# GewelsJI/MVLT

Measured on AMD Instinct MI355X. Metric: image-text pairs/sec/node, PVT-tiny MVLT pre-train step, higher is better.
Workload: dtype bf16

## Files before the change

### mvlt_amd/_lib.py

```python
import ctypes as C
import os

import torch

_HERE = os.path.dirname(os.path.abspath(__file__))
LIB_PATH = os.environ.get("MVLT_HIP_LIB") or os.path.join(_HERE, "libmvlt_hip.so")


class MVLTError(RuntimeError):
    pass


if not os.path.exists(LIB_PATH):
    raise ImportError(f"{LIB_PATH} is missing: build it with `python -m mvlt_amd.build` (hipcc, gfx950). "
                      "mvlt_amd has no CPU or eager fallback.")
lib = C.CDLL(LIB_PATH)

c_int, c_float, c_void_p, c_long = C.c_int, C.c_float, C.c_void_p, C.c_long


class RowMap(C.Structure):
    _fields_ = [(n, c_int) for n in ("mode", "rows_per_batch", "batch_stride", "offset",
                                     "r", "w_in", "tokens_in", "hw_out", "w_out", "c_seg", "h_in")]


class GemmNTArgs(C.Structure):
    _fields_ = [("A", c_void_p), ("B", c_void_p), ("C", c_void_p),
                ("M", c_int), ("N", c_int), ("K", c_int), ("lda", c_int), ("ldb", c_int), ("ldc", c_int),
                ("dtype", c_int), ("out_dtype", c_int),
                ("a_map", RowMap), ("c_map", RowMap),
                ("bias", c_void_p), ("act", c_int), ("H", c_void_p),
                ("row_scale", c_void_p), ("rows_per_scale", c_int), ("R", c_void_p),
                ("col_sum", c_void_p), ("col_sumsq", c_void_p), ("col_copies", c_int), ("split_k", c_int),
                ("post_y", c_void_p), ("post_ld", c_int), ("post_gamma", c_void_p), ("post_beta", c_void_p), ("post_eps", c_float),
                ("post_mean", c_void_p), ("post_rstd", c_void_p), ("r_fp32", c_int)]


class PrepDesc(C.Structure):
    _fields_ = [("src", c_void_p), ("dst", c_void_p), ("kind", c_int), ("R", c_int), ("C", c_int), ("ld_out", c_int),
                ("d0", c_int), ("d1", c_int), ("d2", c_int), ("src_off", c_int), ("ss0", c_int), ("ss1", c_int), ("ss2", c_int),
                ("ds0", c_int), ("ds1", c_int), ("ds2", c_int)]


class GemmTNArgs(C.Structure):
    _fields_ = [("A", c_void_p), ("B", c_void_p), ("C", c_void_p),
                ("M", c_int), ("N1", c_int), ("N2", c_int), ("lda", c_int), ("ldb", c_int), ("ldc", c_int),
                ("dtype", c_int), ("a_map", RowMap), ("b_map", RowMap),
                ("colsum_a", c_void_p), ("splits", c_int), ("colsum_b", c_void_p), ("trans_c", c_int),
                ("c_taps", c_int), ("c_seg", c_int), ("dgrad_wt", c_void_p), ("dgrad_out", c_void_p), ("dgrad_ld", c_int),
                ("partials", c_void_p), ("partials_bytes", c_long), ("defer_fold", c_int), ("c_overwrite", c_int)]


class LayerNormArgs(C.Structure):
    _fields_ = [("x", c_void_p), ("y", c_void_p), ("gamma", c_void_p), ("beta", c_void_p),
                ("mean", c_void_p), ("rstd", c_void_p), ("add", c_void_p), ("add_rows", c_int),
                ("rows", c_int), ("C", c_int), ("ldx", c_int), ("ldy", c_int),
                ("x_map", RowMap), ("y_map", RowMap), ("eps", c_float), ("dtype", c_int), ("y_dtype", c_int),
                ("y2", c_void_p), ("gamma2", c_void_p), ("beta2", c_void_p), ("eps2", c_float), ("mean2", c_void_p), ("rstd2", c_void_p)]


class LayerNormBwdArgs(C.Structure):
    _fields_ = [("dy", c_void_p), ("x", c_void_p), ("dx", c_void_p),
                ("gamma", c_void_p), ("mean", c_void_p), ("rstd", c_void_p),
                ("dgamma", c_void_p), ("dbeta", c_void_p),
                ("rows", c_int), ("C", c_int), ("lddy", c_int), ("ldx", c_int), ("lddx", c_int),
                ("dy_map", RowMap), ("x_map", RowMap), ("dx_map", RowMap),
                ("dx_accumulate", c_int), ("dtype", c_int), ("x_dtype", c_int), ("dx_dtype", c_int),
                ("dx2", c_void_p), ("dx2_scale", c_void_p), ("dx2_rows_per_scale", c_int), ("lddx2", c_int),
                ("dg_copies", c_int), ("dg_copy_stride", c_long)]


class AttnArgs(C.Structure):
    _fields_ = [("Q", c_void_p), ("KV", c_void_p), ("O", c_void_p), ("lse", c_void_p),
                ("B", c_int), ("H", c_int), ("N", c_int), ("M", c_int),
                ("ldq", c_int), ("ldkv", c_int), ("ldo", c_int), ("k_off", c_int), ("v_off", c_int),
                ("scale", c_float), ("dtype", c_int)]


class AttnBwdArgs(C.Structure):
    _fields_ = [("Q", c_void_p), ("KV", c_void_p), ("O", c_void_p), ("dO", c_void_p), ("lse", c_void_p),
                ("dQ", c_void_p), ("dKV", c_void_p),
                ("B", c_int), ("H", c_int), ("N", c_int), ("M", c_int),
                ("ldq", c_int), ("ldkv", c_int), ("ldo", c_int), ("lddkv", c_int),
                ("k_off", c_int), ("v_off", c_int), ("scale", c_float), ("dtype", c_int), ("dkv_dtype", c_int)]


class MlpArgs(C.Structure):
    _fields_ = [("x", c_void_p), ("dy", c_void_p), ("w1", c_void_p), ("wb", c_void_p), ("wc", c_void_p),
                ("b1", c_void_p), ("b2", c_void_p), ("residual", c_void_p), ("row_scale", c_void_p), ("rows_per_scale", c_int),
                ("out", c_void_p), ("h_out", c_void_p), ("dw1", c_void_p), ("db1", c_void_p), ("dw2", c_void_p), ("db2", c_void_p),
                ("M", c_int), ("C", c_int), ("hid", c_int),
                ("ln_x", c_void_p), ("ln_gamma", c_void_p), ("ln_beta", c_void_p), ("ln_eps", c_float),
                ("ln_y", c_void_p), ("ln_mean", c_void_p), ("ln_rstd", c_void_p), ("out_op", c_void_p),
                ("post_gamma", c_void_p), ("post_beta", c_void_p), ("post_eps", c_float),
                ("post_y", c_void_p), ("post_mean", c_void_p), ("post_rstd", c_void_p),
                ("lnb_x", c_void_p), ("lnb_mean", c_void_p), ("lnb_rstd", c_void_p), ("lnb_gamma", c_void_p),
                ("lnb_dx", c_void_p), ("lnb_dx2", c_void_p), ("lnb_dx2_scale", c_void_p), ("lnb_dx2_rows_per_scale", c_int),
                ("lnb_partials", c_void_p), ("partials", c_void_p), ("partials_bytes", c_long), ("defer_fold", c_int)]


STRUCTS = (("mvlt_rowmap", RowMap), ("mvlt_prep_desc", PrepDesc), ("mvlt_gemm_nt_args", GemmNTArgs), ("mvlt_gemm_tn_args", GemmTNArgs),
           ("mvlt_layernorm_args", LayerNormArgs), ("mvlt_layernorm_bwd_args", LayerNormBwdArgs),
           ("mvlt_attn_args", AttnArgs), ("mvlt_attn_bwd_args", AttnBwdArgs), ("mvlt_mlp_args", MlpArgs))

_vp, _i, _l, _f, _u64, _str = c_void_p, c_int, c_long, c_float, C.c_uint64, C.c_char_p
_by_args = lambda cls: (_i, [C.POINTER(cls), _vp])
PROTOTYPES = {
    "mvlt_last_error": (_str, []),
    "mvlt_abi_version": (_i, []),
    "mvlt_last_kernel": (_str, []),
    "mvlt_sizeof": (_i, [_str]),
    "mvlt_gemm_nt": _by_args(GemmNTArgs),
    "mvlt_gemm_tn": _by_args(GemmTNArgs),
    "mvlt_tn_fold_flush": (_i, [_vp, _vp]),
    "mvlt_tn_fold_discard": (_i, [_vp]),
    "mvlt_layernorm_fwd": _by_args(LayerNormArgs),
    "mvlt_layernorm_bwd": _by_args(LayerNormBwdArgs),
    "mvlt_fold_copies": (_i, [_vp, _i, _l, _vp, _i, _i, _vp, _vp]),
    "mvlt_batch_sum": (_i, [_vp, _vp, _i, _i, _i, _l, _i, _i, _vp, _i, _vp]),
    "mvlt_sr_attention_fwd": _by_args(AttnArgs),
    "mvlt_sr_attention_bwd": _by_args(AttnBwdArgs),
    "mvlt_sr_attention_bwd_chunks": (_i, [_i] * 5),
    "mvlt_sr_attention_fwd_streamed": _by_args(AttnArgs),
    "mvlt_sr_attention_bwd_streamed": _by_args(AttnBwdArgs),
    "mvlt_bert_embed_fwd": (_i, [_vp] * 7 + [_f, _vp, _vp, _vp, _i, _i, _i, _f, _i, _vp]),
    "mvlt_bert_embed_bwd": (_i, [_vp] * 7 + [_f] + [_vp] * 7 + [_i, _i, _i, _i, _vp]),
    "mvlt_patchify": (_i, [_vp, _vp, _i, _i, _i, _i, _i, _i, _vp]),
    "mvlt_masked_select": (_i, [_vp, _i, _l, _vp, _vp, _vp]),
    "mvlt_resize_bilinear_tokens": (_i, [_vp, _i, _vp, _i, _i, _i, _i, _i, _i, _i, _vp]),
    "mvlt_resize_bilinear_tokens_multi": (_i, [_vp] * 9 + [_i, _i, _vp]),
    "mvlt_gelu_bwd": (_i, [_vp, _vp, _vp, _l, _i, _vp]),
    "mvlt_loss_compose": (_i, [C.POINTER(c_void_p), C.POINTER(c_float), _vp, _vp, _vp]),
    "mvlt_grid_mask_flags": (_i, [_vp, _i, _i, _i, _i, _i, _u64, _u64, _vp]),
    "mvlt_grid_mask_apply": (_i, [_vp, _vp, _vp, _i, _i, _i, _i, _i, _f, _vp]),
    "mvlt_token_mask": (_i, [_vp, _vp, _vp, _i, _i, _u64, _u64, _i, _vp]),
    "mvlt_keep_mask": (_i, [_vp, _l, _f, _u64, _u64, _vp]),
    "mvlt_droppath_scales": (_i, [_vp, _vp, _i, _i, _u64, _u64, _vp]),
    "mvlt_gather_rows": (_i, [_vp, _vp, _vp, _i, _i, _i, C.POINTER(RowMap), _i, _vp]),
    "mvlt_scatter_rows": (_i, [_vp, _vp, _vp, _i, _i, _i, C.POINTER(RowMap), _i, _i, _vp]),
    "mvlt_cross_entropy_fwd": (_i, [_vp, _vp, _l, _vp, _vp, _vp, _i, _i, _i, _i, _vp]),
    "mvlt_cross_entropy_bwd": (_i, [_vp, _vp, _l, _vp, _vp, _vp, _vp, _i, _i, _i, _i, _i, _i, _vp]),
    "mvlt_smooth_l1_fwd": (_i, [_vp, _vp, _l, _vp, _vp]),
    "mvlt_smooth_l1_bwd": (_i, [_vp, _vp, _l, _vp, _vp, _vp]),
    "mvlt_adamw_step": (_i, [_vp, _vp, _vp, _vp, _vp, _l, _vp, _vp, _vp, _vp]),
    "mvlt_grad_sumsq": (_i, [_vp, _l, _vp, _vp, _i, _vp]),
    "mvlt_clip_coef": (_i, [_vp, _i, _f, _f, _vp, _vp]),
    "mvlt_scale_by_dev": (_i, [_vp, _l, _vp, _vp]),
    "mvlt_cast_bf16": (_i, [_vp, _vp, _l, _vp]),
    "mvlt_row_scale": (_i, [_vp, _vp, _i, _l, _i, _vp, _i, _vp]),
    "mvlt_head_grad_prep": (_i, [_vp, _i, _i, _i, _vp, _vp, _vp, _i, _vp]),
    "mvlt_transpose_cast": (_i, [_vp, _vp, _i, _i, _i, _i, _vp]),
    "mvlt_weight_prep": (_i, [_vp, _vp, _i, _i, _vp, _i, _vp]),
    "mvlt_mlp_fwd": _by_args(MlpArgs),
    "mvlt_mlp_bwd_dx": _by_args(MlpArgs),
    "mvlt_mlp_bwd_dw": _by_args(MlpArgs),
    "mvlt_add_column_sums": (_i, [_vp, _l, _i, _i, _vp, _i, _vp, _vp]),
    "mvlt_col_stats": (_i, [_vp, _i, _l, _i, _vp, _vp, _vp]),
    "mvlt_bn_finalize": (_i, [_vp, _vp, _i, _l, _i, _f, _f, _vp, _vp, _vp, _vp, _vp]),
    "mvlt_bn_norm": (_i, [_vp, _i, _i, _vp, _vp, _vp, _vp, _l, _i, _vp, _i, _i, _vp, _i, _i, _vp]),
    "mvlt_bn_finalize_norm": (_i, [_vp, _i, _vp, _vp, _i, _f, _f, _vp, _vp, _vp, _vp, _vp, _vp, _l, _i, _vp, _i, _i, _vp, _i, _vp]),
    "mvlt_bn_bwd_reduce": (_i, [_vp, _i, _vp, _i, _i, _vp, _vp, _l, _i, _vp, _vp, _i, _vp]),
    "mvlt_bn_bwd_apply": (_i, [_vp, _i, _vp, _i, _i, _vp, _vp, _vp, _vp, _vp, _l, _i, _vp, _i, _vp, _vp, _i, _i, _vp]),
    "mvlt_ew_mul": (_i, [_vp, _i, _vp, _i, _vp, _i, _vp, _i, _i, _l, _i, _i, _vp, _i, _i, _vp]),
    "mvlt_ew_mul3_bwd": (_i, [_vp, _i, _vp, _vp, _vp, _i, _i, _vp, _vp, _vp, _l, _i, _i, _vp]),
    "mvlt_upsample_fwd": (_i, [_vp, _i, _i, _i, _i, _i, _i, _vp, _i, _i, _i, _vp]),
    "mvlt_upsample_bwd": (_i, [_vp, _i, _i, _i, _i, _i, _i, _i, _vp, _i, _i, _i, _i, _vp]),
    "mvlt_upsample_l1_fwd": (_i, [_vp, _i, _i, _i, _i, _i, _i, _vp, _vp, _vp]),
    "mvlt_upsample_l1_bwd": (_i, [_vp, _i, _i, _i, _i, _i, _i, _vp, _vp, _vp, _i, _i, _vp]),
}
EXPORTS = list(PROTOTYPES)
for _name, (_res, _args) in PROTOTYPES.items():
    _fn = getattr(lib, _name)
    _fn.restype, _fn.argtypes = _res, _args

ABI_VERSION = 8
if lib.mvlt_abi_version() != ABI_VERSION:
    raise ImportError(f"ABI mismatch: {LIB_PATH} is version {lib.mvlt_abi_version()}, the binding is version {ABI_VERSION} (stale build? run python -m mvlt_amd.build)")
for _name, _cls in STRUCTS:
    _n = lib.mvlt_sizeof(_name.encode())
    if _n != C.sizeof(_cls):
        raise ImportError(f"ABI mismatch for {_name}: library says {_n} bytes, binding has {C.sizeof(_cls)}")

EXT_PROTOTYPES = {
    "mvlt_ext_version": (_i, []),
    "mvlt_step_gate": (_i, [_vp, _i, _f, _f, _vp, _vp, _vp]),
    "mvlt_adamw_step_gated": (_i, [_vp, _vp, _vp, _vp, _vp, _l, _vp, _vp, _vp, _vp]),
}
for _name, (_res, _args) in EXT_PROTOTYPES.items():
    if not hasattr(lib, _name):
        raise ImportError(f"{LIB_PATH} does not export {_name} (include/mvlt_hip_ext.h): stale build? run python -m mvlt_amd.build")
    _fn = getattr(lib, _name)
    _fn.restype, _fn.argtypes = _res, _args

EXT_VERSION = 1
if lib.mvlt_ext_version() != EXT_VERSION:
    raise ImportError(f"extension mismatch: {LIB_PATH} is version {lib.mvlt_ext_version()}, the binding is version {EXT_VERSION} (stale build? run python -m mvlt_amd.build)")

EMA_PROTOTYPES = {
    "mvlt_ema_version": (_i, []),
    "mvlt_ema_update": (_i, [_vp, _vp, _vp, _l, _f, _f, _vp, _vp]),
    "mvlt_ema_update_buffers": (_i, [_vp, _i, _f, _f, _vp]),
}
for _name, (_res, _args) in EMA_PROTOTYPES.items():
    if not hasattr(lib, _name):
        raise ImportError(f"{LIB_PATH} does not export {_name} (include/mvlt_hip_ema.h): stale build? run python -m mvlt_amd.build")
    _fn = getattr(lib, _name)
    _fn.restype, _fn.argtypes = _res, _args

EMA_VERSION = 1
if lib.mvlt_ema_version() != EMA_VERSION:
    raise ImportError(f"EMA entry points mismatch: {LIB_PATH} is version {lib.mvlt_ema_version()}, the binding is version {EMA_VERSION} (stale build? run python -m mvlt_amd.build)")

class GemmPlan(C.Structure):
    _fields_ = [("family", c_int), ("tp", c_int * 6), ("grid", c_int * 3), ("block", c_int), ("lds", c_int),
                ("ns_flags", c_int), ("nbuf", c_int), ("per_split", c_int), ("t1", c_int), ("t2", c_int), ("splits", c_int),
                ("swap_operands", c_int), ("fold", c_int), ("fold_grid", c_int), ("partials_need", c_long)]


class AttnPlan(C.Structure):
    _fields_ = [("family", c_int), ("tp", c_int * 4), ("grid", c_int), ("block", c_int), ("lds", c_int), ("nq_chunks", c_int), ("q_per_wg", c_int)]


class MlpPlan(C.Structure):
    _fields_ = [("family", c_int), ("tp", c_int * 2), ("grid", c_int), ("block", c_int), ("lds", c_int), ("m_per_split", c_int), ("splits", c_int), ("ny", c_int),
                ("fold", c_int), ("fold_grid", c_int * 2), ("partials_need", c_long)]


PLAN_STRUCTS = (("mvlt_gemm_plan", GemmPlan), ("mvlt_attn_plan", AttnPlan), ("mvlt_mlp_plan", MlpPlan))
PLAN_PROTOTYPES = {
    "mvlt_plan_version": (_i, []),
    "mvlt_gemm_nt_plan": (_i, [C.POINTER(GemmNTArgs), C.POINTER(GemmPlan)]),
    "mvlt_gemm_tn_plan": (_i, [C.POINTER(GemmTNArgs), C.POINTER(GemmPlan)]),
    "mvlt_gemm_plan_name": (_i, [C.POINTER(GemmPlan), _str, C.c_size_t]),
    "mvlt_gemm_plan_sizeof": (_i, []),
    "mvlt_sr_attention_fwd_plan": (_i, [C.POINTER(AttnArgs), _i, C.POINTER(AttnPlan)]),
    "mvlt_sr_attention_bwd_plan": (_i, [C.POINTER(AttnBwdArgs), _i, C.POINTER(AttnPlan)]),
    "mvlt_attn_plan_name": (_i, [C.POINTER(AttnPlan), _str, C.c_size_t]),
    "mvlt_attn_plan_sizeof": (_i, []),
    "mvlt_mlp_fwd_plan": (_i, [C.POINTER(MlpArgs), C.POINTER(MlpPlan)]),
    "mvlt_mlp_bwd_dx_plan": (_i, [C.POINTER(MlpArgs), C.POINTER(MlpPlan)]),
    "mvlt_mlp_bwd_dw_plan": (_i, [C.POINTER(MlpArgs), C.POINTER(MlpPlan)]),
    "mvlt_mlp_plan_name": (_i, [C.POINTER(MlpPlan), _str, C.c_size_t]),
    "mvlt_mlp_plan_sizeof": (_i, []),
}
for _name, (_res, _args) in PLAN_PROTOTYPES.items():
    if not hasattr(lib, _name):
        raise ImportError(f"{LIB_PATH} does not export {_name} (include/mvlt_hip_plan.h): stale build? run python -m mvlt_amd.build")
    _fn = getattr(lib, _name)
    _fn.restype, _fn.argtypes = _res, _args

PLAN_VERSION = 3
_plan_sizes = [(n, getattr(lib, n + "_sizeof")(), C.sizeof(c)) for n, c in PLAN_STRUCTS]
if lib.mvlt_plan_version() != PLAN_VERSION or any(have != want for _, have, want in _plan_sizes):
    raise ImportError(f"plan entry points mismatch: {LIB_PATH} is version {lib.mvlt_plan_version()}, the binding is version {PLAN_VERSION}; (struct, bytes in the library, "
                      f"bytes in the binding): {_plan_sizes} (stale build? run python -m mvlt_amd.build)")

OPT_PROTOTYPES = {
    "mvlt_opt_version": (_i, []),
    "mvlt_adamw_step_groups": (_i, [_vp, _vp, _vp, _vp, _vp, _l, _vp, _vp, _vp, _i, _vp, _vp, _vp]),
}
for _name, (_res, _args) in OPT_PROTOTYPES.items():
    if not hasattr(lib, _name):
        raise ImportError(f"{LIB_PATH} does not export {_name} (include/mvlt_hip_opt.h): stale build? run python -m mvlt_amd.build")
    _fn = getattr(lib, _name)
    _fn.restype, _fn.argtypes = _res, _args

OPT_VERSION = 1
if lib.mvlt_opt_version() != OPT_VERSION:
    raise ImportError(f"optimizer entry points mismatch: {LIB_PATH} is version {lib.mvlt_opt_version()}, the binding is version {OPT_VERSION} (stale build? run python -m mvlt_amd.build)")

LAMB_PROTOTYPES = {
    "mvlt_lamb_version": (_i, []),
    "mvlt_lamb_check_tables": (_i, [_vp, _i, _vp, _i, _l, _i]),
    "mvlt_lamb_moments": (_i, [_vp, _vp, _vp, _vp, _l, _vp, _vp, _i, _vp, _i, _vp, _i, _vp, _vp, _vp, _vp]),
    "mvlt_lamb_fold": (_i, [_vp, _i, _vp, _i, _vp, _i, _i, _vp, _vp, _vp]),
    "mvlt_lamb_apply": (_i, [_vp, _vp, _vp, _vp, _l, _vp, _vp, _i, _vp, _i, _vp, _i, _vp, _vp, _vp]),
}
for _name, (_res, _args) in LAMB_PROTOTYPES.items():
    if not hasattr(lib, _name):
        raise ImportError(f"{LIB_PATH} does not export {_name} (include/mvlt_hip_lamb.h): stale build? run python -m mvlt_amd.build")
    _fn = getattr(lib, _name)
    _fn.restype, _fn.argtypes = _res, _args

LAMB_VERSION = 1
if lib.mvlt_lamb_version() != LAMB_VERSION:
    raise ImportError(f"LAMB entry points mismatch: {LIB_PATH} is version {lib.mvlt_lamb_version()}, the binding is version {LAMB_VERSION} (stale build? run python -m mvlt_amd.build)")

LOSS_PROTOTYPES = {
    "mvlt_loss_version": (_i, []),
    "mvlt_ce_smooth_fwd": (_i, [_vp, _vp, _l, _f, _vp, _vp, _vp, _vp, _i, _i, _i, _i, _vp]),
    "mvlt_ce_smooth_bwd": (_i, [_vp, _vp, _l, _f, _vp, _vp, _vp, _vp, _vp, _i, _i, _i, _i, _i, _i, _vp]),
}
for _name, (_res, _args) in LOSS_PROTOTYPES.items():
    if not hasattr(lib, _name):
        raise ImportError(f"{LIB_PATH} does not export {_name} (include/mvlt_hip_loss.h): stale build? run python -m mvlt_amd.build")
    _fn = getattr(lib, _name)
    _fn.restype, _fn.argtypes = _res, _args

LOSS_VERSION = 1
if lib.mvlt_loss_version() != LOSS_VERSION:
    raise ImportError(f"loss entry points mismatch: {LIB_PATH} is version {lib.mvlt_loss_version()}, the binding is version {LOSS_VERSION} (stale build? run python -m mvlt_amd.build)")

INGEST_PROTOTYPES = {
    "mvlt_ingest_version": (_i, []),
    "mvlt_image_ingest": (_i, [_vp, _i, _vp, _vp, _vp, _vp, _i, _i, _i, _i, _f, _vp]),
    "mvlt_image_ingest_resize": (_i, [_vp, _i, _i, _vp, _vp, _vp, _vp, _vp, _vp, _vp, _i, _i, _i, _i, _f, _vp]),
    "mvlt_flip_flags": (_i, [_vp, _i, _f, _u64, _u64, _vp]),
}
for _name, (_res, _args) in INGEST_PROTOTYPES.items():
    if not hasattr(lib, _name):
        raise ImportError(f"{LIB_PATH} does not export {_name} (include/mvlt_hip_ingest.h): stale build? run python -m mvlt_amd.build")
    _fn = getattr(lib, _name)
    _fn.restype, _fn.argtypes = _res, _args

INGEST_VERSION = 1
if lib.mvlt_ingest_version() != INGEST_VERSION:
    raise ImportError(f"ingest entry points mismatch: {LIB_PATH} is version {lib.mvlt_ingest_version()}, the binding is version {INGEST_VERSION} (stale build? run python -m mvlt_amd.build)")

DT = {torch.bfloat16: 0, torch.float32: 1}


def last_kernel():
    s = lib.mvlt_last_kernel().decode()
    s = s.replace("(anonymous namespace)::", "")
    if s.startswith("void "):
        s = s[5:]
    depth = 0
    for i, ch in enumerate(s):
        depth += ch == "<"
        depth -= ch == ">"
        if ch == "(" and depth == 0:
            return s[:i]
    return s


def check(rc, what):
    if rc != 0:
        raise MVLTError(f"{what} failed ({rc}): {lib.mvlt_last_error().decode()}")


_raw_stream, _cur_device = torch._C._cuda_getCurrentRawStream, torch._C._cuda_getDevice


def stream_ptr():
    return _raw_stream(_cur_device())


def ptr(t):
    if t is None:
        return None
    if not t.is_cuda:
        raise MVLTError("mvlt_amd ops need CUDA/HIP tensors (no CPU fallback)")
    return t.data_ptr()


def rowmap(rows_per_batch=0, batch_stride=0, offset=0):
    return RowMap(0, rows_per_batch, batch_stride, offset, 0, 0, 0, 0, 0, 0, 0)


def patchmap(r, w_in, tokens_in, hw_out, w_out, c_seg):
    return RowMap(1, 0, 0, 0, r, w_in, tokens_in, hw_out, w_out, c_seg, 0)


def conv3map(h, w, tokens_in, c_seg):
    return RowMap(2, 0, 0, 0, 3, w, tokens_in, h * w, w, c_seg, h)
```

### mvlt_amd/build.py

```python
import concurrent.futures
import os
import subprocess
import sys

HERE = os.path.dirname(os.path.abspath(__file__))
CSRC = os.path.join(HERE, "csrc")
OBJ = os.path.join(HERE, "csrc", "_obj")
LIB = os.path.join(HERE, "libmvlt_hip.so")
ARCH = "gfx950"
FLAGS = ["--offload-arch=" + ARCH, "-O3", "-std=c++17", "-fPIC", "-ffp-contract=fast", "-Wno-unused-result"]
EXTRA = {f: ["-fno-slp-vectorize"] for f in ("mlp_fused.hip", "mlp_pipe.hip", "mlp_wgrad.hip")}


def _sources():
    return sorted(f for f in os.listdir(CSRC) if f.endswith(".hip"))


def source_hash():
    import hashlib
    h = hashlib.sha256()
    files = sorted(os.path.join(CSRC, f) for f in os.listdir(CSRC) if f.endswith((".hip", ".h", ".inc")))
    files += [os.path.join(HERE, "..", "include", h) for h in ("mvlt_hip.h", "mvlt_hip_ext.h", "mvlt_hip_ema.h", "mvlt_hip_plan.h", "mvlt_hip_opt.h", "mvlt_hip_lamb.h", "mvlt_hip_loss.h", "mvlt_hip_ingest.h")]
    for f in files:
        h.update(os.path.basename(f).encode())
        h.update(open(f, "rb").read())
    return h.hexdigest()[:16]


def _deps_mtime():
    hdrs = [os.path.join(CSRC, f) for f in os.listdir(CSRC) if f.endswith((".h", ".inc"))]
    hdrs += [os.path.join(HERE, "..", "include", h) for h in ("mvlt_hip.h", "mvlt_hip_ext.h", "mvlt_hip_ema.h", "mvlt_hip_plan.h", "mvlt_hip_opt.h", "mvlt_hip_lamb.h", "mvlt_hip_loss.h", "mvlt_hip_ingest.h")]
    return max(os.path.getmtime(h) for h in hdrs)


def _compile(src, force, verbose):
    s = os.path.join(CSRC, src)
    o = os.path.join(OBJ, src[:-4] + ".o")
    if not force and os.path.exists(o) and os.path.getmtime(o) >= max(os.path.getmtime(s), _deps_mtime()):
        return o
    cmd = ["hipcc", *FLAGS, *EXTRA.get(src, []), "-c", s, "-o", o]
    if verbose:
        print(" ".join(cmd), flush=True)
    r = subprocess.run(cmd, capture_output=True, text=True)
    if r.returncode != 0:
        raise RuntimeError(f"hipcc failed for {src}:\n{r.stdout}\n{r.stderr}")
    return o


def build(force=False, verbose=False):
    os.makedirs(OBJ, exist_ok=True)
    srcs = _sources()
    with concurrent.futures.ThreadPoolExecutor(max_workers=min(8, len(srcs))) as ex:
        objs = list(ex.map(lambda s: _compile(s, force, verbose), srcs))
    if force or not os.path.exists(LIB) or any(os.path.getmtime(o) > os.path.getmtime(LIB) for o in objs):
        cmd = ["hipcc", "--offload-arch=" + ARCH, "-shared", "-fPIC", *objs, "-o", LIB]
        if verbose:
            print(" ".join(cmd), flush=True)
        r = subprocess.run(cmd, capture_output=True, text=True)
        if r.returncode != 0:
            raise RuntimeError(f"link failed:\n{r.stdout}\n{r.stderr}")
    return LIB


if __name__ == "__main__":
    print(build(force="--force" in sys.argv, verbose="--verbose" in sys.argv or True))
```

### mvlt_amd/csrc/gemm.hip

```cpp
#include "gemm_common.h"
#include <map>
#include <mutex>

namespace {

constexpr int FOLD_MAX = 32;
struct FoldDesc { const bf16* part; float* C; int splits, N1, N2, ldc, wg0; };
struct FoldBatch { FoldDesc d[FOLD_MAX]; int n, total_wgs; };

__device__ __forceinline__ void tn_fold_body(const bf16* __restrict__ part, int splits, int N1, int N2, float* __restrict__ C, int ldc, int blk) {
  __shared__ float red[8][32][9];
  const int eg = threadIdx.x & 31, sk = threadIdx.x >> 5;
  const long g = (long)blk * 32 + eg;
  const long per = (long)N1 * N2;
  const bool ok = g * 8 < per;
  float s[8] = {0.f, 0.f, 0.f, 0.f, 0.f, 0.f, 0.f, 0.f};
  if (ok) {
    for (int z = sk; z < splits; z += 8) {
      const bf16x8 v = __builtin_bit_cast(bf16x8, ld_g<MVLT_NT_LD>((const u32x4*)(part + (size_t)z * per + g * 8)));
#pragma unroll
      for (int e = 0; e < 8; ++e) s[e] += (float)v[e];
    }
  }
#pragma unroll
  for (int e = 0; e < 8; ++e) red[sk][eg][e] = s[e];
  __syncthreads();
  if (sk == 0 && ok) {
#pragma unroll
    for (int k = 1; k < 8; ++k)
#pragma unroll
      for (int e = 0; e < 8; ++e) s[e] += red[k][eg][e];
    const int n1 = (int)((g * 8) / N2), n2 = (int)((g * 8) - (long)n1 * N2);
    float* dst = C + (long)n1 * ldc + n2;
    const f32x4 a = *(const f32x4*)dst, b = *(const f32x4*)(dst + 4);
    *(f32x4*)dst = f32x4{a[0] + s[0], a[1] + s[1], a[2] + s[2], a[3] + s[3]};
    *(f32x4*)(dst + 4) = f32x4{b[0] + s[4], b[1] + s[5], b[2] + s[6], b[3] + s[7]};
  }
}

__global__ __launch_bounds__(256) void tn_fold_kernel(const bf16* __restrict__ part, int splits, int N1, int N2, float* __restrict__ C, int ldc) {
  tn_fold_body(part, splits, N1, N2, C, ldc, blockIdx.x);
}
__global__ __launch_bounds__(256) void tn_fold_multi_kernel(FoldBatch b) {
  int i = 0;
#pragma unroll 1
  for (int k = 1; k < b.n; ++k) if ((int)blockIdx.x >= b.d[k].wg0) i = k;
  const FoldDesc& d = b.d[i];
  tn_fold_body(d.part, d.splits, d.N1, d.N2, d.C, d.ldc, (int)blockIdx.x - d.wg0);
}

struct FoldPending {
  FoldBatch b = {};
  long used = 0;
  hipStream_t stream = nullptr;
  hipEvent_t ev = nullptr;
};
std::mutex g_fold_mu;
std::map<const void*, FoldPending> g_fold;
int fold_wgs(const FoldDesc& d) { return (int)(((long)d.N1 * d.N2 / 8 + 31) / 32); }
void fold_flush_locked(FoldPending& f, hipStream_t reader, bool order_reader) {
  if (f.b.n > 0) {
    f.b.total_wgs = f.b.d[f.b.n - 1].wg0 + fold_wgs(f.b.d[f.b.n - 1]);
    MVLT_LAUNCH(tn_fold_multi_kernel, dim3((unsigned)f.b.total_wgs), dim3(256), 0, f.stream, f.b);
    if (order_reader && reader != f.stream) {
      if (!f.ev) (void)hipEventCreateWithFlags(&f.ev, hipEventDisableTiming);
      if (f.ev && hipEventRecord(f.ev, f.stream) == hipSuccess) (void)hipStreamWaitEvent(reader, f.ev, 0);
    }
  }
  f.b.n = 0;
  f.used = 0;
}
bf16* fold_acquire(const mvlt_gemm_tn_args& a, long need, hipStream_t s, int room = 1) {
  if (!a.partials || ((uintptr_t)a.partials & 15) || need > a.partials_bytes) return nullptr;
  std::lock_guard<std::mutex> lk(g_fold_mu);
  FoldPending& f = g_fold[a.partials];
  bool flush = f.b.n > 0 && (!a.defer_fold || f.stream != s || f.b.n + room > FOLD_MAX || f.used + need > a.partials_bytes);
  const float* c_lo = a.C;
  const float* c_hi = a.C + (size_t)(a.N1 - 1) * a.ldc + a.N2;
  for (int i = 0; i < f.b.n && !flush; ++i) {
    const FoldDesc& d = f.b.d[i];
    const float* d_lo = d.C;
    const float* d_hi = d.C + (size_t)(d.N1 - 1) * d.ldc + d.N2;
    if (c_lo < d_hi && d_lo < c_hi) flush = true;
  }
  if (flush) fold_flush_locked(f, s, true);
  f.stream = s;
  if (!a.defer_fold) return (bf16*)a.partials;
  return (bf16*)((char*)a.partials + f.used);
}
void fold_launch(const mvlt_gemm_tn_args& a, const bf16* part, int splits, hipStream_t s) {
  const long groups = (long)a.N1 * a.N2 / 8;
  if (!a.defer_fold) {
    MVLT_LAUNCH(tn_fold_kernel, dim3((unsigned)((groups + 31) / 32)), dim3(256), 0, s, part, splits, a.N1, a.N2, a.C, a.ldc);
    return;
  }
  std::lock_guard<std::mutex> lk(g_fold_mu);
  FoldPending& f = g_fold[a.partials];
  FoldDesc& d = f.b.d[f.b.n];
  d.part = part; d.C = a.C; d.splits = splits; d.N1 = a.N1; d.N2 = a.N2; d.ldc = a.ldc;
  d.wg0 = f.b.n == 0 ? 0 : f.b.d[f.b.n - 1].wg0 + fold_wgs(f.b.d[f.b.n - 1]);
  ++f.b.n;
  f.used += ((long)splits * a.N1 * a.N2 * 2 + 255) & ~255L;
}

int launch_nt(const mvlt_gemm_plan& p, const mvlt_gemm_nt_args& a, hipStream_t s) {
  switch (p.family) {
    case MVLT_GEMM_NT_F32:
    case MVLT_GEMM_NT_DMA: return mvlt_launch_nt_dma(p, a, s);
    case MVLT_GEMM_NT_P8: return mvlt_launch_nt_p8(p, a, s);
    case MVLT_GEMM_NT_CONV3: return mvlt_launch_nt_conv3(p, a, s);
  }
  return no_instantiation("mvlt_gemm_nt", p);
}

int launch_tn(const mvlt_gemm_plan& p, const mvlt_gemm_tn_args& a, hipStream_t s) {
  const char* const who = "mvlt_gemm_tn";
  mvlt_gemm_tn_args k = a;
  if (p.swap_operands) {
    k.A = a.B; k.B = a.A; k.lda = a.ldb; k.ldb = a.lda; k.N1 = a.N2; k.N2 = a.N1;
    k.colsum_a = a.colsum_b; k.colsum_b = a.colsum_a;
  }
  bf16* const part = p.fold ? fold_acquire(a, p.partials_need, s) : nullptr;
  if (p.fold && !part) { mvlt_set_error("%s: the planned %ld bytes of partial tiles do not fit the scratch", who, p.partials_need); return MVLT_ERR_ARG; }
  auto launch = [&]() -> int {
    switch (p.family) {
      case MVLT_GEMM_TN_PLAIN:
      case MVLT_GEMM_TN_DMA: return mvlt_launch_tn_dma(p, k, part, s);
      case MVLT_GEMM_TN_P8: return mvlt_launch_tn_p8(p, k, part, s);
      case MVLT_GEMM_TN_CONV3: return mvlt_launch_tn_conv3(p, k, part, s);
    }
    return no_instantiation(who, p);
  };
  const int e = launch();
  if (e != MVLT_OK || !p.fold) return e;
  fold_launch(a, part, p.splits, s);
  return mvlt_check_launch(who);
}
}

extern "C" int mvlt_gemm_nt(const mvlt_gemm_nt_args* a, void* stream) {
  mvlt_gemm_plan p;
  MVLT_REQUIRE(a, "mvlt_gemm_nt: null operand");
  if (int e = plan_gemm_nt(*a, p)) return e;
  return p.family == MVLT_GEMM_NONE ? MVLT_OK : launch_nt(p, *a, (hipStream_t)stream);
}

extern "C" int mvlt_gemm_tn(const mvlt_gemm_tn_args* a, void* stream) {
  mvlt_gemm_plan p;
  MVLT_REQUIRE(a, "mvlt_gemm_tn: null operand");
  if (int e = plan_gemm_tn(*a, p)) return e;
  return p.family == MVLT_GEMM_NONE ? MVLT_OK : launch_tn(p, *a, (hipStream_t)stream);
}

extern "C" int mvlt_plan_version(void) { return MVLT_PLAN_VERSION; }
extern "C" int mvlt_gemm_plan_sizeof(void) { return (int)sizeof(mvlt_gemm_plan); }
extern "C" int mvlt_gemm_nt_plan(const mvlt_gemm_nt_args* a, mvlt_gemm_plan* plan) {
  MVLT_REQUIRE(a && plan, "mvlt_gemm_nt_plan: null argument");
  return plan_gemm_nt(*a, *plan);
}
extern "C" int mvlt_gemm_tn_plan(const mvlt_gemm_tn_args* a, mvlt_gemm_plan* plan) {
  MVLT_REQUIRE(a && plan, "mvlt_gemm_tn_plan: null argument");
  return plan_gemm_tn(*a, *plan);
}
extern "C" int mvlt_gemm_plan_name(const mvlt_gemm_plan* plan, char* buf, size_t n) {
  MVLT_REQUIRE(plan && buf && n > 0, "mvlt_gemm_plan_name: null argument");
  return plan_kernel_name(*plan, buf, n);
}

bf16* mvlt_fold_acquire_ext(const mvlt_gemm_tn_args& a, long need, hipStream_t s, int descriptors) { return fold_acquire(a, need, s, descriptors); }
void mvlt_fold_launch_ext(const mvlt_gemm_tn_args& a, const bf16* part, int splits, hipStream_t s) { fold_launch(a, part, splits, s); }

extern "C" int mvlt_tn_fold_discard(const void* partials) {
  std::lock_guard<std::mutex> lk(g_fold_mu);
  for (auto& kv : g_fold)
    if (!partials || kv.first == partials) { kv.second.b.n = 0; kv.second.used = 0; }
  return MVLT_OK;
}

extern "C" int mvlt_tn_fold_flush(const void* partials, void* stream) {
  std::lock_guard<std::mutex> lk(g_fold_mu);
  for (auto& kv : g_fold)
    if (!partials || kv.first == partials) fold_flush_locked(kv.second, (hipStream_t)stream, true);
  return mvlt_check_launch("mvlt_tn_fold_flush");
}
```

### mvlt_amd/csrc/gemm_common.h

```cpp
#pragma once
#include "common.h"
#include "gemm_plan.h"
#include <type_traits>
#include "../../include/mvlt_hip.h"

int mvlt_launch_nt_dma(const mvlt_gemm_plan& p, const mvlt_gemm_nt_args& a, hipStream_t s);
int mvlt_launch_nt_p8(const mvlt_gemm_plan& p, const mvlt_gemm_nt_args& a, hipStream_t s);
int mvlt_launch_nt_conv3(const mvlt_gemm_plan& p, const mvlt_gemm_nt_args& a, hipStream_t s);
int mvlt_launch_tn_dma(const mvlt_gemm_plan& p, const mvlt_gemm_tn_args& k, bf16* part, hipStream_t s);
int mvlt_launch_tn_p8(const mvlt_gemm_plan& p, const mvlt_gemm_tn_args& k, bf16* part, hipStream_t s);
int mvlt_launch_tn_conv3(const mvlt_gemm_plan& p, const mvlt_gemm_tn_args& k, bf16* part, hipStream_t s);

namespace {

constexpr int BM = 128;
constexpr int NTHREADS = 256;
constexpr int ROW_BYTES = 128;
constexpr int CHUNKS = 8;

template <typename T> struct Elem;
template <> struct Elem<bf16> { static constexpr int BK = 64; static constexpr int PER_CHUNK = 8; };
template <> struct Elem<float> { static constexpr int BK = 32; static constexpr int PER_CHUNK = 4; };

__device__ __forceinline__ int swz(int row, int chunk) { return chunk ^ ((row >> 1) & 7); }

__device__ __forceinline__ RowMap to_rowmap(const mvlt_rowmap& m) {
  RowMap r;
  r.mode = m.mode; r.rows_per_batch = m.rows_per_batch; r.batch_stride = m.batch_stride; r.offset = m.offset;
  r.r = m.r; r.w_in = m.w_in; r.tokens_in = m.tokens_in; r.hw_out = m.hw_out; r.w_out = m.w_out; r.c_seg = m.c_seg;
  r.h_in = m.h_in;
  return r;
}

__device__ __forceinline__ void mma16(f32x4& acc, const u32x4& a0, const u32x4& a1, const u32x4& b0, const u32x4& b1, bf16*) {
  acc = __builtin_amdgcn_mfma_f32_16x16x32_bf16(__builtin_bit_cast(bf16x8, a0), __builtin_bit_cast(bf16x8, b0), acc, 0, 0, 0);
  (void)a1; (void)b1;
}
__device__ __forceinline__ void mma16(f32x4& acc, const u32x4& a0, const u32x4& a1, const u32x4& b0, const u32x4& b1, float*) {
  f32x4 fa0 = __builtin_bit_cast(f32x4, a0), fa1 = __builtin_bit_cast(f32x4, a1);
  f32x4 fb0 = __builtin_bit_cast(f32x4, b0), fb1 = __builtin_bit_cast(f32x4, b1);
#pragma unroll
  for (int j = 0; j < 4; ++j) acc = __builtin_amdgcn_mfma_f32_16x16x4f32(fa0[j], fb0[j], acc, 0, 0, 0);
#pragma unroll
  for (int j = 0; j < 4; ++j) acc = __builtin_amdgcn_mfma_f32_16x16x4f32(fa1[j], fb1[j], acc, 0, 0, 0);
}

typedef _Float16 f16x8 __attribute__((ext_vector_type(8)));
__device__ __forceinline__ void round_f16_8(float (&v)[8]) {
#pragma unroll
  for (int e = 0; e < 8; ++e) v[e] = (float)(_Float16)__builtin_amdgcn_fmed3f(v[e], -65504.f, 65504.f);
}
template <bool NTF> __device__ __forceinline__ void store_f16_8(void* base, long ix, const float (&v)[8]) {
  f16x8 o;
#pragma unroll
  for (int e = 0; e < 8; ++e) o[e] = (_Float16)v[e];
  st_g<NTF>((f16x8*)((_Float16*)base + ix), o);
}
template <typename T> __device__ __forceinline__ void store_out(void* base, long idx, float v, int out_fp32) {
  if (out_fp32) ((float*)base)[idx] = v; else ((bf16*)base)[idx] = (bf16)v;
}
__device__ __forceinline__ float load_out(const void* base, long idx, int out_fp32) {
  return out_fp32 ? ((const float*)base)[idx] : (float)((const bf16*)base)[idx];
}

template <typename T, int BN>
__device__ __forceinline__ void nt_epilogue(const mvlt_gemm_nt_args& p, f32x4 (&acc)[4][BN / 32], char* smem, int m0, int n0,
                                            int wave, int lane) {
  constexpr int WN = BN / 2;
  constexpr int TN_ = WN / 16;
  const int wm = wave >> 1, wn = wave & 1;
  const int fr = lane & 15, fg = lane >> 4;
  const RowMap cmap = to_rowmap(p.c_map);
  const int ofp32 = p.out_dtype;
  constexpr int LDW = WN + 4;
  constexpr int CPR = WN / 8;
  constexpr int RPI = 64 / CPR;
  float* stage = (float*)smem + wave * 32 * LDW;
  const bool vec_ok = (p.ldc % 8 == 0) && (((uintptr_t)p.C & 15) == 0) && (!p.R || ((uintptr_t)p.R & 15) == 0) &&
                      (!p.H || ((uintptr_t)p.H & 15) == 0);
  const int nc_lane = n0 + wn * WN + (lane % CPR) * 8;
  float bias8[8];
#pragma unroll
  for (int e = 0; e < 8; ++e) bias8[e] = 0.f;
  if (p.bias && p.split_k <= 1) {
    if (nc_lane + 8 <= p.N && (((uintptr_t)p.bias & 15) == 0)) {
      f32x4 b0 = *(const f32x4*)(p.bias + nc_lane), b1 = *(const f32x4*)(p.bias + nc_lane + 4);
#pragma unroll
      for (int e = 0; e < 4; ++e) { bias8[e] = b0[e]; bias8[4 + e] = b1[e]; }
    } else {
#pragma unroll
      for (int e = 0; e < 8; ++e) if (nc_lane + e < p.N) bias8[e] = p.bias[nc_lane + e];
    }
  }
  float cs8[8], cq8[8];
#pragma unroll
  for (int e = 0; e < 8; ++e) { cs8[e] = 0.f; cq8[e] = 0.f; }
#pragma unroll
  for (int half = 0; half < 2; ++half) {
    __builtin_amdgcn_wave_barrier();
#pragma unroll
    for (int ii = 0; ii < 2; ++ii)
#pragma unroll
      for (int j = 0; j < TN_; ++j)
#pragma unroll
        for (int r = 0; r < 4; ++r) stage[(ii * 16 + 4 * fg + r) * LDW + j * 16 + fr] = acc[half * 2 + ii][j][r];
    __builtin_amdgcn_fence(__ATOMIC_RELEASE, "wavefront");
    __builtin_amdgcn_wave_barrier();
    __builtin_amdgcn_fence(__ATOMIC_ACQUIRE, "wavefront");
    if (p.split_k > 1) {
      const int col = n0 + wn * WN + lane;
      if (lane < WN && col < p.N) {
        const float bv = (p.bias && blockIdx.y == 0) ? p.bias[col] : 0.f;
        for (int r = 0; r < 32; ++r) {
          const int m = m0 + wm * 64 + half * 32 + r;
          if (m < p.M) atomicAdd((float*)p.C + (long)m * p.ldc + col, stage[r * LDW + lane] + bv);
        }
      }
      continue;
    }
#pragma unroll
    for (int it = 0; it < 32 / RPI; ++it) {
      const int rl = it * RPI + lane / CPR;
      const int ch = lane % CPR;
      const int m = m0 + wm * 64 + half * 32 + rl;
      const int nc = n0 + wn * WN + ch * 8;
      if (m >= p.M || nc >= p.N) continue;
      f32x4 v0 = *(const f32x4*)(stage + rl * LDW + ch * 8), v1 = *(const f32x4*)(stage + rl * LDW + ch * 8 + 4);
      float v[8] = {v0[0], v0[1], v0[2], v0[3], v1[0], v1[1], v1[2], v1[3]};
      int seg_rows = 0, ncol = nc;
      if (cmap.mode == 1) {
        int seg = nc / cmap.c_seg;
        ncol = nc - seg * cmap.c_seg;
        seg_rows = rowmap_seg(cmap, seg);
      }
      const long idx = (rowmap_base(cmap, m) + seg_rows) * p.ldc + ncol;
      const bool full = vec_ok && (nc + 8 <= p.N);
      const float rs = p.row_scale ? p.row_scale[m / p.rows_per_scale] : 1.0f;
#pragma unroll
      for (int e = 0; e < 8; ++e) v[e] += bias8[e];
      if (full) {
        auto load8 = [&](const void* base, float* o) {
          if (ofp32) {
            f32x4 a = *(const f32x4*)((const float*)base + idx), b = *(const f32x4*)((const float*)base + idx + 4);
#pragma unroll
            for (int e = 0; e < 4; ++e) { o[e] = a[e]; o[4 + e] = b[e]; }
          } else {
            bf16x8 a = *(const bf16x8*)((const bf16*)base + idx);
#pragma unroll
            for (int e = 0; e < 8; ++e) o[e] = (float)a[e];
          }
        };
        auto store8 = [&](void* base, const float* o) {
          if (ofp32) {
            st_g<MVLT_NT_GEMM>((f32x4*)((float*)base + idx), f32x4{o[0], o[1], o[2], o[3]});
            st_g<MVLT_NT_GEMM>((f32x4*)((float*)base + idx + 4), f32x4{o[4], o[5], o[6], o[7]});
          } else {
            bf16x8 a;
#pragma unroll
            for (int e = 0; e < 8; ++e) a[e] = (bf16)o[e];
            st_g<MVLT_NT_GEMM>((bf16x8*)((bf16*)base + idx), a);
          }
        };
        if (p.act == 1) {
          if (p.H) store8(p.H, v);
#pragma unroll
          for (int e = 0; e < 8; e += 2) {
            const f32x2 gv = gelu_erf2(f32x2{v[e], v[e + 1]});
            v[e] = gv[0]; v[e + 1] = gv[1];
          }
        } else if (p.act == 2) {
          float h8[8];
          load8(p.H, h8);
#pragma unroll
          for (int e = 0; e < 8; e += 2) {
            const f32x2 dv = gelu_erf_grad2(f32x2{h8[e], h8[e + 1]});
            v[e] *= dv[0]; v[e + 1] *= dv[1];
          }
        }
        if (p.row_scale) {
#pragma unroll
          for (int e = 0; e < 8; ++e) v[e] *= rs;
        }
        if (p.R) {
          float r8[8];
          load8(p.R, r8);
#pragma unroll
          for (int e = 0; e < 8; ++e) v[e] += r8[e];
        }
        if (p.col_sum) {
#pragma unroll
          for (int e = 0; e < 8; ++e) { cs8[e] += v[e]; cq8[e] += v[e] * v[e]; }
        }
        store8(p.C, v);
      } else {
        for (int e = 0; e < 8; ++e) {
          if (nc + e >= p.N) break;
          float x = v[e];
          if (p.act == 1) {
            if (p.H) store_out<T>(p.H, idx + e, x, ofp32);
            x = gelu_erf(x);
          } else if (p.act == 2) {
            x *= gelu_erf_grad(load_out(p.H, idx + e, ofp32));
          }
          x *= rs;
          if (p.R) x += load_out(p.R, idx + e, ofp32);
          if (p.col_sum) { cs8[e] += x; cq8[e] += x * x; }
          store_out<T>(p.C, idx + e, x, ofp32);
        }
      }
    }
  }
  if (p.col_sum) {
#pragma unroll
    for (int off = CPR; off < 64; off <<= 1)
#pragma unroll
      for (int e = 0; e < 8; ++e) { cs8[e] += __shfl_xor(cs8[e], off); cq8[e] += __shfl_xor(cq8[e], off); }
    __builtin_amdgcn_fence(__ATOMIC_RELEASE, "wavefront");
    __builtin_amdgcn_wave_barrier();
    if (lane < CPR) {
#pragma unroll
      for (int e = 0; e < 8; ++e) { stage[lane * 8 + e] = cs8[e]; stage[WN + lane * 8 + e] = cq8[e]; }
    }
    __builtin_amdgcn_fence(__ATOMIC_RELEASE, "wavefront");
    __builtin_amdgcn_wave_barrier();
    __builtin_amdgcn_fence(__ATOMIC_ACQUIRE, "wavefront");
    const int col = n0 + wn * WN + lane;
    const long cpy = p.col_copies > 1 ? (long)((m0 / BM) % p.col_copies) * p.N : 0;
    if (lane < WN && col < p.N) {
      atomicAdd(&p.col_sum[cpy + col], stage[lane]);
      atomicAdd(&p.col_sumsq[cpy + col], stage[WN + lane]);
    }
  }
}

__device__ __forceinline__ int fdiv24(int m, int d, float inv) {
  int q = (int)((float)m * inv);
  int r = m - q * d;
  return q + (r >= d) - (r < 0);
}
template <int BN, int EPIX, int TM = 4, int NWN = 2, bool FULL = false>
__device__ __forceinline__ void nt_epilogue_lean(const mvlt_gemm_nt_args& p, f32x4 (&acc)[TM][BN / 32], char* smem, int m0, int n0,
                                                 int wave, int lane) {
  static_assert(NWN == 2 || EPIX != 8, "the LayerNorm epilogue pairs the two waves of a row: 2 x 2 wave grids only");
  constexpr bool SCAT = (EPIX == 6 || EPIX == 7);
  constexpr bool POST = EPIX == 8;
  constexpr int EPI = EPIX == 6 ? 1 : (EPIX == 7 || EPIX == 8) ? 2 : EPIX;
  constexpr int WN = BN / 2;
  constexpr int TN_ = WN / 16;
  constexpr int LDW = WN + 4;
  constexpr int CPR = WN / 8;
  constexpr int RPI = 64 / CPR;
  constexpr int NIT = 32 / RPI;
  const int wm = wave / NWN, wn = wave % NWN;
  const int fr = lane & 15, fg = lane >> 4;
  const int ofp32 = (EPI == 3 || EPI == 4) ? 0 : p.out_dtype;
  const int rfp32 = (EPI == 2 && !POST) ? (ofp32 | p.r_fp32) : ofp32;
  float* stage = (float*)smem + wave * 32 * LDW;
  const int ch = lane % CPR;
  const int nc = n0 + wn * WN + ch * 8;
  const bool col_ok = FULL || nc < p.N;
  float bias8[8];
#pragma unroll
  for (int e = 0; e < 8; ++e) bias8[e] = 0.f;
  if (p.bias && col_ok) {
    if (!FULL && nc + 8 > p.N) {
#pragma unroll
      for (int e = 0; e < 8; ++e) if (nc + e < p.N) bias8[e] = p.bias[nc + e];
    } else if (((uintptr_t)p.bias & 15) == 0) {
      f32x4 b0 = *(const f32x4*)(p.bias + nc), b1 = *(const f32x4*)(p.bias + nc + 4);
#pragma unroll
      for (int e = 0; e < 4; ++e) { bias8[e] = b0[e]; bias8[4 + e] = b1[e]; }
    } else {
#pragma unroll
      for (int e = 0; e < 8; ++e) bias8[e] = p.bias[nc + e];
    }
  }
  constexpr int NH = TM / 2;
  const int m_first = m0 + wm * (TM * 16) + lane / CPR;
  const int rpb = p.c_map.rows_per_batch;
  const float inv_rpb = rpb > 0 ? 1.0f / (float)rpb : 0.f;
  int seg_rows = 0, ncol = nc;
  float inv_hw = 0.f, inv_w = 0.f;
  if constexpr (SCAT) {
    const int seg = nc / p.c_map.c_seg;
    ncol = nc - seg * p.c_map.c_seg;
    const int di = seg / p.c_map.r;
    seg_rows = di * p.c_map.w_in + (seg - di * p.c_map.r);
    inv_hw = 1.0f / (float)p.c_map.hw_out;
    inv_w = 1.0f / (float)p.c_map.w_out;
  }
  const float inv_rps = (EPI == 2 && p.rows_per_scale > 0) ? 1.0f / (float)p.rows_per_scale : 0.f;
  float cs8[8], cq8[8];
  if (EPI == 5) {
#pragma unroll
    for (int e = 0; e < 8; ++e) { cs8[e] = 0.f; cq8[e] = 0.f; }
  }
  long idx[2][NIT];
  bool ok[2][NIT];
  float rs[2][NIT];
  u32x4 raw[2][NIT][2];
  auto request = [&](int half) {
    const int sl = half & 1;
#pragma unroll
    for (int it = 0; it < NIT; ++it) {
      const int m = m_first + half * 32 + it * RPI;
      ok[sl][it] = FULL || (m < p.M && col_ok);
      const int mm = (FULL || ok[sl][it]) ? m : 0;
      long phys = mm;
      if constexpr (SCAT) {
// ... 500 lines not shown
```

### mvlt_amd/csrc/gemm_nt_dma.hip

```cpp
#include "gemm_common.h"

namespace {

template <typename T, int BN>
__global__ __launch_bounds__(NTHREADS) void gemm_nt_kernel(mvlt_gemm_nt_args p, int nbuf) {
  constexpr int BK = Elem<T>::BK;
  constexpr int PC = Elem<T>::PER_CHUNK;
  constexpr int WN = BN / 2;
  constexpr int TN_ = WN / 16;
  constexpr int A_ITERS = BM * CHUNKS / NTHREADS;
  constexpr int B_ITERS = BN * CHUNKS / NTHREADS;
  extern __shared__ __attribute__((aligned(16))) char smem[];
  char* sA = smem;
  char* sB = smem + nbuf * BM * ROW_BYTES;

  const int tid = threadIdx.x, lane = tid & 63, wave = tid >> 6;
  const int wm = wave >> 1, wn = wave & 1;
  const int tiles_m = (p.M + BM - 1) / BM;
  const int tiles_n = (p.N + BN - 1) / BN;
  const int bid = blockIdx.x;
  const int xcd = bid & 7, slot = bid >> 3;
  const int tile_m = (slot / tiles_n) * 8 + xcd, tile_n = slot % tiles_n;
  if (tile_m >= tiles_m) return;
  const int m0 = tile_m * BM, n0 = tile_n * BN;
  const RowMap amap = to_rowmap(p.a_map);

  const int chunk = tid & 7;
  const int row_in = tid >> 3;
  const T* Ag = (const T*)p.A;
  const T* Bg = (const T*)p.B;

  long a_base[A_ITERS];
  bool a_ok[A_ITERS];
  int a_y[A_ITERS], a_x[A_ITERS];
#pragma unroll
  for (int i = 0; i < A_ITERS; ++i) {
    int m = m0 + row_in + 32 * i;
    a_ok[i] = m < p.M;
    a_base[i] = a_ok[i] ? rowmap_base(amap, m) : 0;
    a_y[i] = 0; a_x[i] = 0;
    if (amap.mode == 2 && a_ok[i]) rowmap_yx(amap, m, a_y[i], a_x[i]);
  }
  long b_base[B_ITERS];
  bool b_ok[B_ITERS];
#pragma unroll
  for (int i = 0; i < B_ITERS; ++i) {
    int n = n0 + row_in + 32 * i;
    b_ok[i] = n < p.N;
    b_base[i] = b_ok[i] ? (long)n * p.ldb : 0;
  }

  u32x4 ra[A_ITERS], rb[B_ITERS];
  auto gload = [&](int kt) {
    const int k = kt * BK + chunk * PC;
    const bool k_ok = k < p.K;
    int seg_rows = 0, kk = k, seg = 0;
    if (amap.mode != 0) {
      seg = k / amap.c_seg;
      kk = k - seg * amap.c_seg;
      if (amap.mode == 1) seg_rows = rowmap_seg(amap, seg);
    }
#pragma unroll
    for (int i = 0; i < A_ITERS; ++i) {
      u32x4 v = {0u, 0u, 0u, 0u};
      bool ok = a_ok[i] && k_ok;
      int off = seg_rows;
      if (amap.mode == 2) ok = ok && rowmap_nb(amap, seg, a_y[i], a_x[i], off);
      if (ok) v = *(const u32x4*)(Ag + (a_base[i] + off) * p.lda + kk);
      ra[i] = v;
    }
#pragma unroll
    for (int i = 0; i < B_ITERS; ++i) {
      u32x4 v = {0u, 0u, 0u, 0u};
      if (b_ok[i] && k_ok) v = *(const u32x4*)(Bg + b_base[i] + k);
      rb[i] = v;
    }
  };
  auto lstore = [&](int buf) {
#pragma unroll
    for (int i = 0; i < A_ITERS; ++i) {
      int r = row_in + 32 * i;
      *(u32x4*)(sA + buf * BM * ROW_BYTES + r * ROW_BYTES + swz(r, chunk) * 16) = ra[i];
    }
#pragma unroll
    for (int i = 0; i < B_ITERS; ++i) {
      int r = row_in + 32 * i;
      *(u32x4*)(sB + buf * BN * ROW_BYTES + r * ROW_BYTES + swz(r, chunk) * 16) = rb[i];
    }
  };

  f32x4 acc[4][TN_];
#pragma unroll
  for (int i = 0; i < 4; ++i)
#pragma unroll
    for (int j = 0; j < TN_; ++j) acc[i][j] = f32x4{0.f, 0.f, 0.f, 0.f};

  const int nk = (p.K + BK - 1) / BK;
  gload(0);
  lstore(0);
  __syncthreads();
  const int fr = lane & 15, fg = lane >> 4;
  for (int kt = 0; kt < nk; ++kt) {
    const int buf = kt & 1;
    if (kt + 1 < nk) gload(kt + 1);
    const char* a_s = sA + buf * BM * ROW_BYTES + (wm * 64) * ROW_BYTES;
    const char* b_s = sB + buf * BN * ROW_BYTES + (wn * WN) * ROW_BYTES;
    constexpr int KSTEPS = (sizeof(T) == 2) ? 2 : 1;
    constexpr int CPS = (sizeof(T) == 2) ? 1 : 2;
#pragma unroll
    for (int ks = 0; ks < KSTEPS; ++ks) {
      u32x4 fa[4][2], fb[TN_][2];
#pragma unroll
      for (int i = 0; i < 4; ++i) {
        int r = i * 16 + fr;
        int rr = wm * 64 + r;
#pragma unroll
        for (int c = 0; c < CPS; ++c) {
          int ch = (sizeof(T) == 2) ? (ks * 4 + fg) : (fg * 2 + c);
          fa[i][c] = *(const u32x4*)(a_s + r * ROW_BYTES + swz(rr, ch) * 16);
        }
        if (CPS == 1) fa[i][1] = fa[i][0];
      }
#pragma unroll
      for (int j = 0; j < TN_; ++j) {
        int r = j * 16 + fr;
        int rr = wn * WN + r;
#pragma unroll
        for (int c = 0; c < CPS; ++c) {
          int ch = (sizeof(T) == 2) ? (ks * 4 + fg) : (fg * 2 + c);
          fb[j][c] = *(const u32x4*)(b_s + r * ROW_BYTES + swz(rr, ch) * 16);
        }
        if (CPS == 1) fb[j][1] = fb[j][0];
      }
#pragma unroll
      for (int i = 0; i < 4; ++i)
#pragma unroll
        for (int j = 0; j < TN_; ++j) mma16(acc[i][j], fa[i][0], fa[i][1], fb[j][0], fb[j][1], (T*)nullptr);
    }
    if (kt + 1 < nk) lstore(buf ^ 1);
    __syncthreads();
  }

  nt_epilogue<T, BN>(p, acc, smem, m0, n0, wave, lane);
}

template <int BN, int AMODE, int EPI, int BK, int BMT = BM>
__global__ __launch_bounds__(NTHREADS, BMT == 256 ? 2 : 1) void gemm_nt_dma_kernel(mvlt_gemm_nt_args p, int ns_flags) {
  const int ns = ns_flags & 0xff;
  const bool early = (ns_flags & 0x100) != 0;
  constexpr int ROWB = BK * 2;
  constexpr int CH = BK / 8;
  constexpr int RPL = NTHREADS / CH;
  constexpr int WN = BN / 2, TN_ = WN / 16;
  constexpr int WM = BMT / 2, TM_ = WM / 16;
  constexpr int A_ITERS = BMT * CH / NTHREADS;
  constexpr int B_ITERS = BN * CH / NTHREADS;
  constexpr int LPT = A_ITERS + B_ITERS;
  constexpr int STAGE = (BMT + BN) * ROWB;
  auto swzk = [](int row, int chunk) { return CH == 8 ? (chunk ^ ((row >> 1) & 7)) : (chunk ^ ((0 - (row >> 2)) & 3)); };
  extern __shared__ __attribute__((aligned(16))) char smem[];

  const int tid = threadIdx.x, lane = tid & 63, wave = __builtin_amdgcn_readfirstlane(tid >> 6);
  const int wm = wave >> 1, wn = wave & 1;
  const int tiles_m = (p.M + BMT - 1) / BMT;
  const int tiles_n = (p.N + BN - 1) / BN;
  const int bid = blockIdx.x;
  const int xcd = bid & 7, bslot = bid >> 3;
  const int tile_m = (bslot / tiles_n) * 8 + xcd, tile_n = bslot % tiles_n;
  if (tile_m >= tiles_m) return;
  const int m0 = tile_m * BMT, n0 = tile_n * BN;
  const RowMap amap = to_rowmap(p.a_map);
  const unsigned smem_lds = (unsigned)(uintptr_t)smem;

  const int row_in = tid / CH;
  const int chunk = swzk(row_in, tid % CH);
  const char* zsrc = (const char*)g_zero_page + ((tid * 16 + (bid & 15) * 4096) & 65535);

  const char* a_ptr[A_ITERS];
  bool a_ok[A_ITERS];
  int a_y[A_ITERS], a_x[A_ITERS];
#pragma unroll
  for (int i = 0; i < A_ITERS; ++i) {
    int m = m0 + row_in + RPL * i;
    a_ok[i] = m < p.M;
    RowIt it = row_init(amap, a_ok[i] ? m : 0);
    int phys;
    if constexpr (AMODE == 0) phys = it.b * amap.batch_stride + amap.offset + it.x;
    else if constexpr (AMODE == 1) phys = it.b * amap.tokens_in + (it.y * amap.r) * amap.w_in + it.x * amap.r;
    else phys = it.b * amap.tokens_in + it.y * amap.w_in + it.x;
    a_y[i] = it.y; a_x[i] = it.x;
    a_ptr[i] = (const char*)p.A + (unsigned long long)(unsigned)phys * (2u * (unsigned)p.lda);
  }
  const char* b_ptr[B_ITERS];
  bool b_ok[B_ITERS];
#pragma unroll
  for (int i = 0; i < B_ITERS; ++i) {
    int n = n0 + row_in + RPL * i;
    b_ok[i] = n < p.N;
    b_ptr[i] = (const char*)p.B + (unsigned long long)(unsigned)(b_ok[i] ? n : 0) * (2u * (unsigned)p.ldb);
  }

  const int nk_all = (p.K + BK - 1) / BK;
  const int nsplit = p.split_k > 1 ? p.split_k : 1;
  const int kt_per = (nk_all + nsplit - 1) / nsplit;
  const int kt0 = blockIdx.y * kt_per;
  int kpos = kt0 * BK + chunk * 8, seg = 0, kk = kpos;
  if constexpr (AMODE != 0) { seg = kk / amap.c_seg; kk -= seg * amap.c_seg; }
  auto issue = [&](int slot) {
    const bool k_ok = kpos < p.K;
    int off_bytes = (AMODE == 0 ? kpos : kk) * 2, tdy = 0, tdx = 0;
    if constexpr (AMODE == 1) off_bytes += rowmap_seg(amap, seg) * (2 * p.lda);
    if constexpr (AMODE == 2) {
      const int dy = seg / 3;
      tdy = dy - 1; tdx = seg - dy * 3 - 1;
      off_bytes += (tdy * amap.w_in + tdx) * (2 * p.lda);
    }
#pragma unroll
    for (int i = 0; i < A_ITERS; ++i) {
      bool ok = a_ok[i] && k_ok;
      if constexpr (AMODE == 2) ok = ok && (unsigned)(a_y[i] + tdy) < (unsigned)amap.h_in && (unsigned)(a_x[i] + tdx) < (unsigned)amap.w_in;
      glds16(ok ? a_ptr[i] + off_bytes : zsrc, __builtin_amdgcn_readfirstlane(smem_lds + slot * STAGE + (i * NTHREADS + wave * 64) * 16));
    }
#pragma unroll
    for (int i = 0; i < B_ITERS; ++i)
      glds16((b_ok[i] && k_ok) ? b_ptr[i] + kpos * 2 : zsrc,
             __builtin_amdgcn_readfirstlane(smem_lds + slot * STAGE + BMT * ROWB + (i * NTHREADS + wave * 64) * 16));
    kpos += BK;
    if constexpr (AMODE != 0) {
      kk += BK;
      while (kk >= amap.c_seg) { kk -= amap.c_seg; ++seg; }
    }
  };

  f32x4 acc[TM_][TN_];
#pragma unroll
  for (int i = 0; i < TM_; ++i)
#pragma unroll
    for (int j = 0; j < TN_; ++j) acc[i][j] = f32x4{0.f, 0.f, 0.f, 0.f};

  const int nk = min(kt_per, nk_all - kt0);
  if (nk <= 0) return;
  const int fr = lane & 15, fg = lane >> 4;
  for (int st = 0; st < (early ? ns : ns - 1) && st < nk; ++st) issue(st);
  if (ns == 1 && !early) issue(0);
  int slot = 0, islot = early ? 0 : ns - 1;
  for (int kt = 0; kt < nk; ++kt) {
    const int ahead = min(nk - 1 - kt, early ? ns - 1 : ns - 2);
    if (ahead >= 4) asm volatile("s_waitcnt vmcnt(%0) lgkmcnt(0)" ::"n"(4 * LPT) : "memory");
    else if (ahead == 3) asm volatile("s_waitcnt vmcnt(%0) lgkmcnt(0)" ::"n"(3 * LPT) : "memory");
    else if (ahead == 2) asm volatile("s_waitcnt vmcnt(%0) lgkmcnt(0)" ::"n"(2 * LPT) : "memory");
    else if (ahead == 1) asm volatile("s_waitcnt vmcnt(%0) lgkmcnt(0)" ::"n"(LPT) : "memory");
    else asm volatile("s_waitcnt vmcnt(0) lgkmcnt(0)" ::: "memory");
    __builtin_amdgcn_s_barrier();
    asm volatile("" ::: "memory");
    if (!early) {
      if (ns > 1 && kt + ns - 1 < nk) issue(islot);
      islot = islot + 1 >= ns ? 0 : islot + 1;
    }
    const char* a_s = smem + slot * STAGE + (wm * WM) * ROWB;
    const char* b_s = smem + slot * STAGE + BMT * ROWB + (wn * WN) * ROWB;
    slot = slot + 1 >= ns ? 0 : slot + 1;
    constexpr int KS = BK / 32;
    u32x4 fa[KS][TM_], fb[KS][TN_];
#pragma unroll
    for (int ks = 0; ks < KS; ++ks) {
#pragma unroll
      for (int i = 0; i < TM_; ++i) {
        int r = i * 16 + fr;
        fa[ks][i] = *(const u32x4*)(a_s + r * ROWB + swzk(wm * WM + r, ks * 4 + fg) * 16);
      }
#pragma unroll
      for (int j = 0; j < TN_; ++j) {
        int r = j * 16 + fr;
        fb[ks][j] = *(const u32x4*)(b_s + r * ROWB + swzk(wn * WN + r, ks * 4 + fg) * 16);
      }
    }
    if (early) {
      asm volatile("s_waitcnt lgkmcnt(0)" ::: "memory");
      __builtin_amdgcn_s_barrier();
      asm volatile("" ::: "memory");
      if (kt + ns < nk) issue(islot);
      islot = islot + 1 >= ns ? 0 : islot + 1;
    }
#pragma unroll
    for (int ks = 0; ks < KS; ++ks) {
      __builtin_amdgcn_sched_barrier(0);
#pragma unroll
      for (int i = 0; i < TM_; ++i)
#pragma unroll
        for (int j = 0; j < TN_; ++j) mma16(acc[i][j], fa[ks][i], fa[ks][i], fb[ks][j], fb[ks][j], (bf16*)nullptr);
    }
  }
  __syncthreads();
  static_assert(BMT == BM || (BN != 192 && EPI != 0), "the 256-row tile carries the lean epilogues only");
  if constexpr (BN == 192) nt_epilogue_192<EPI>(p, acc, smem, m0, n0, wave, lane);
  else if constexpr (EPI == 0) nt_epilogue<bf16, BN>(p, acc, smem, m0, n0, wave, lane);
  else nt_epilogue_lean<BN, EPI, TM_>(p, acc, smem, m0, n0, wave, lane);
}

}

int mvlt_launch_nt_dma(const mvlt_gemm_plan& p, const mvlt_gemm_nt_args& a, hipStream_t s) {
  const char* const who = "mvlt_gemm_nt";
  MVLT_PLAN_LAUNCH_HEAD;
#define NT_F32(BN_) MVLT_CASE(false, (gemm_nt_kernel<float, BN_>), (MVLT_GEMM_NT_F32, BN_), a, p.nbuf)
#define NT_DMA(BN_, AM_, EPI_, BK_) MVLT_CASE(false, (gemm_nt_dma_kernel<BN_, AM_, EPI_, BK_>), (MVLT_GEMM_NT_DMA, BN_, AM_, EPI_, BK_), a, p.ns_flags)
#define NT_DMA_EPIS(BN_, AM_) NT_DMA(BN_, AM_, 1, 64) NT_DMA(BN_, AM_, 2, 64) NT_DMA(BN_, AM_, 3, 64) NT_DMA(BN_, AM_, 4, 64) \
                              NT_DMA(BN_, AM_, 5, 64) NT_DMA(BN_, AM_, 6, 64) NT_DMA(BN_, AM_, 7, 64) NT_DMA(BN_, AM_, 0, 64)
  switch (key) {
    NT_DMA(64, 0, 8, 64) NT_DMA(128, 0, 8, 64)
    NT_DMA(192, 0, 1, 64) NT_DMA(192, 0, 5, 64) NT_DMA(192, 2, 1, 64) NT_DMA(192, 2, 5, 64)
    NT_DMA_EPIS(64, 0) NT_DMA_EPIS(64, 1) NT_DMA_EPIS(64, 2)
    NT_DMA(128, 0, 3, 32) NT_DMA(128, 0, 4, 32)
    NT_DMA_EPIS(128, 0) NT_DMA_EPIS(128, 1) NT_DMA_EPIS(128, 2)
    NT_F32(64) NT_F32(128)
  }
  return no_instantiation(who, p);
}
```

### mvlt_amd/csrc/gemm_plan.h

```cpp
#pragma once
#include <stdint.h>
#include <stdio.h>
#include "../../include/mvlt_hip_plan.h"
#include "plan_common.h"
#ifndef MVLT_NT_EARLY_DEFAULT
#define MVLT_NT_EARLY_DEFAULT 0x100
#endif

namespace mvlt_plan {

constexpr int BM = 128;
constexpr int NTHREADS = 256;
constexpr int ROW_BYTES = 128;
constexpr int TBK = 64;
constexpr int TN_ROWB_BF16 = (TBK + 8) * 2, TN_ROWB_F32 = (TBK + 4) * 4;
constexpr int TN_TILE64_BYTES = TBK * 64 * 2;

inline bool al16(const void* p) { return ((uintptr_t)p & 15) == 0; }
inline int cdiv(int a, int b) { return (a + b - 1) / b; }
inline int xcd_grid(int n) { return n >= 8 ? 8 * cdiv(n, 8) : n; }
inline int xcd_round(int splits) { return splits >= 8 ? (splits + 4) / 8 * 8 : splits; }

struct Split { int splits, per; };
inline Split split_even(int splits, int ktiles) {
  if (splits > ktiles) splits = ktiles;
  if (splits < 1) splits = 1;
  const int per = cdiv(ktiles, splits);
  return {cdiv(ktiles, per), per};
}
inline Split split_choose(int want, int ktiles, int min_tiles, bool round_first) {
  if (round_first) { want = xcd_round(want); if (want > 4096) want = 4096; }
  if (want > ktiles / min_tiles) want = ktiles / min_tiles;
  if (!round_first) want = xcd_round(want);
  return split_even(want, ktiles);
}
inline int fold_workgroups(int N1, int N2) { return (int)(((long)N1 * N2 / 8 + 31) / 32); }
inline bool scratch_fits(const mvlt_gemm_tn_args& a, long need) { return a.partials && al16(a.partials) && need <= a.partials_bytes; }
inline void plan_fold(const mvlt_gemm_tn_args& a, mvlt_gemm_plan& p) {
  p.fold = 1;
  p.partials_need = (long)p.splits * a.N1 * a.N2 * 2;
  p.fold_grid = fold_workgroups(a.N1, a.N2);
}

inline int check_rowmap(const mvlt_rowmap& m, const char* who) {
  if (m.mode == 0) {
    MVLT_REQUIRE(m.rows_per_batch >= 0, "%s: rows_per_batch < 0", who);
  } else if (m.mode == 1) {
    MVLT_REQUIRE(m.r > 0 && m.w_in > 0 && m.tokens_in > 0 && m.hw_out > 0 && m.w_out > 0 && m.c_seg > 0 && m.c_seg % 16 == 0,
                 "%s: bad patch map (c_seg must be a positive multiple of 16)", who);
  } else if (m.mode == 2) {
    MVLT_REQUIRE(m.r == 3 && m.w_in > 0 && m.h_in > 0 && m.tokens_in >= m.h_in * m.w_in && m.hw_out == m.h_in * m.w_in &&
                 m.w_out == m.w_in && m.c_seg > 0 && m.c_seg % 8 == 0, "%s: bad 3x3 neighbourhood map", who);
  } else {
    MVLT_REQUIRE(false, "%s: unknown rowmap mode %d", who, m.mode);
  }
  return MVLT_OK;
}

inline void set_tp(mvlt_gemm_plan& p, int family, int t0, int t1 = 0, int t2 = 0, int t3 = 0, int t4 = 0, int t5 = 0) {
  p.family = family;
  p.tp[0] = t0; p.tp[1] = t1; p.tp[2] = t2; p.tp[3] = t3; p.tp[4] = t4; p.tp[5] = t5;
}
inline void set_launch(mvlt_gemm_plan& p, int gx, int gy, int gz, int block, long lds) {
  p.grid[0] = gx; p.grid[1] = gy; p.grid[2] = gz; p.block = block; p.lds = (int)lds;
}
inline void plan_nt_p8(const mvlt_gemm_nt_args& a, mvlt_gemm_plan& p, int epi, int hm, int hn0, int hn1, int rag) {
  const int bmt = 64 * hm, bnt = 64 * (hn0 + hn1);
  const int lds_loop = 2 * (2 * (2 * hm * 16) + 64 * (hn0 + hn1)) * 128, lds_epi = 8 * 32 * (16 * (hn0 + hn1) + 4) * 4;
  set_tp(p, MVLT_GEMM_NT_P8, epi, hm, hn0, hn1, rag);
  set_launch(p, 8 * cdiv(cdiv(a.M, bmt), 8) * cdiv(a.N, bnt), 1, 1, 512, lds_loop > lds_epi ? lds_loop : lds_epi);
}

}

inline int plan_gemm_nt(const mvlt_gemm_nt_args& a, mvlt_gemm_plan& p) {
  using namespace mvlt_plan;
  p = mvlt_gemm_plan{};
  MVLT_REQUIRE(a.A && a.B && a.C, "mvlt_gemm_nt: null operand");
  MVLT_REQUIRE(a.M >= 0 && a.N > 0 && a.K > 0, "mvlt_gemm_nt: bad shape M=%d N=%d K=%d", a.M, a.N, a.K);
  MVLT_REQUIRE(a.dtype == 0 || a.dtype == 1, "mvlt_gemm_nt: dtype must be 0 (bf16) or 1 (fp32)");
  const int pc = a.dtype == 0 ? 8 : 4;
  MVLT_REQUIRE(a.K % pc == 0 && a.lda % pc == 0 && a.ldb % pc == 0, "mvlt_gemm_nt: K/lda/ldb must be multiples of %d elements (16 B)", pc);
  MVLT_REQUIRE(al16(a.A) && al16(a.B), "mvlt_gemm_nt: A/B must be 16-byte aligned");
  MVLT_REQUIRE(a.act >= 0 && a.act <= 2, "mvlt_gemm_nt: bad act");
  MVLT_REQUIRE(a.act != 2 || a.H, "mvlt_gemm_nt: act=2 (gelu') needs H");
  MVLT_REQUIRE(!a.row_scale || a.rows_per_scale > 0, "mvlt_gemm_nt: row_scale needs rows_per_scale");
  MVLT_REQUIRE((a.col_sum == nullptr) == (a.col_sumsq == nullptr), "mvlt_gemm_nt: col_sum and col_sumsq come together");
  MVLT_REQUIRE(a.split_k <= 1 || (a.dtype == 0 && a.out_dtype == 1 && a.act == 0 && !a.H && !a.R && !a.row_scale && !a.col_sum &&
                                  a.c_map.mode == 0 && a.split_k <= 64),
               "mvlt_gemm_nt: split_k needs bf16 operands, fp32 C (zeroed by the caller) and a plain epilogue (A may be gathered)");
  MVLT_REQUIRE(a.col_copies >= 0, "mvlt_gemm_nt: col_copies < 0");
  MVLT_REQUIRE(!a.r_fp32 || (a.R && a.R != a.C && a.dtype == 0 && a.out_dtype == 0 && a.act == 0 && !a.col_sum && !a.post_y && a.split_k <= 1 && a.c_map.mode == 0 &&
                             a.N % 8 == 0 && a.ldc % 8 == 0 && (((uintptr_t)a.C | (uintptr_t)a.R) & 15) == 0 && a.M < (1 << 24)),
               "mvlt_gemm_nt: r_fp32 (fp32 residual beside a bf16 C) exists in the residual epilogue of the bf16 LDS-DMA kernels only (plain c_map, N % 8 == 0, 16-byte aligned C / R)");
  MVLT_REQUIRE(a.out_dtype >= 0 && a.out_dtype <= 2, "mvlt_gemm_nt: out_dtype is 0 (bf16), 1 (fp32) or 2 (fp16, with col_sum only)");
  MVLT_REQUIRE(a.out_dtype != 2 || (a.dtype == 0 && a.col_sum && a.act == 0 && !a.R && !a.row_scale && a.split_k <= 1 && a.c_map.mode == 0 && a.N % 8 == 0 &&
                                    a.ldc % 8 == 0 && al16(a.C) && a.M < (1 << 24)),
               "mvlt_gemm_nt: fp16 output exists in the column-statistics epilogue of the bf16 LDS-DMA kernels only (plain c_map, N % 8 == 0, 16-byte aligned C)");
  if (int e = check_rowmap(a.a_map, "mvlt_gemm_nt a_map")) return e;
  if (int e = check_rowmap(a.c_map, "mvlt_gemm_nt c_map")) return e;
  MVLT_REQUIRE(a.a_map.mode == 0 || a.K == a.a_map.r * a.a_map.r * a.a_map.c_seg, "mvlt_gemm_nt: gather K != r*r*c_seg");
  MVLT_REQUIRE(a.c_map.mode == 0 || a.N == a.c_map.r * a.c_map.r * a.c_map.c_seg, "mvlt_gemm_nt: scatter N != r*r*c_seg");
  MVLT_REQUIRE(a.c_map.mode != 2, "mvlt_gemm_nt: the 3x3 map is a gather only (its dgrad is a gather with flipped taps)");
  MVLT_REQUIRE(!a.post_y || (a.dtype == 0 && a.split_k <= 1),
               "mvlt_gemm_nt: post_y needs the bf16 LDS-DMA path (no fp32 operands, no split_k)");
  if (a.M == 0) return MVLT_OK;
  const int tiles_m = cdiv(a.M, BM);
  const bool narrow = a.N <= 64;
  const int bn = narrow ? 64 : 128;
  const int tiles_n = cdiv(a.N, bn);
  const int ksplit = a.split_k > 1 ? a.split_k : 1;
  const long stage = (long)4 * 32 * (bn / 2 + 4) * sizeof(float);
  const int gx = 8 * cdiv(tiles_m, 8) * tiles_n;
  if (a.dtype != 0) {
    p.nbuf = a.K <= 32 ? 1 : 2;
    const long lds = (long)p.nbuf * (BM + bn) * ROW_BYTES;
    set_tp(p, MVLT_GEMM_NT_F32, bn);
    set_launch(p, gx, ksplit, 1, NTHREADS, lds < stage ? stage : lds);
    return MVLT_OK;
  }
  int epi = 0;
  const bool plain_epi = a.act == 0 && !a.R && !a.row_scale && !a.col_sum && !a.H && a.c_map.mode == 0;
  const bool lean_ok = (a.c_map.mode == 0 || (a.c_map.mode == 1 && a.c_map.c_seg % 8 == 0)) && a.split_k <= 1 && (a.N % 8 == 0 || plain_epi) && a.ldc % 8 == 0 && al16(a.C) &&
                       (!a.R || al16(a.R)) && (!a.H || al16(a.H)) && a.M < (1 << 24);
  if (lean_ok && a.c_map.mode == 1) {
    if (a.act == 0 && !a.col_sum && !a.R && !a.row_scale) epi = 6;
    else if (a.act == 0 && !a.col_sum && a.R) epi = 7;
  } else if (lean_ok) {
    if (a.act == 1 && !a.R && !a.row_scale && !a.col_sum && a.out_dtype == 0) epi = 3;
    else if (a.act == 2 && !a.R && !a.row_scale && !a.col_sum && a.out_dtype == 0) epi = 4;
    else if (a.act == 0 && a.R && !a.col_sum) epi = 2;
    else if (a.act == 0 && !a.R && !a.row_scale && a.col_sum) epi = 5;
    else if (a.act == 0 && !a.R && !a.row_scale && !a.col_sum) epi = 1;
  }
  const int bk = (!narrow && a.a_map.mode == 0 && (epi == 3 || epi == 4) && a.K <= 512) ? 32 : 64;
  const int nk = bk == 32 ? cdiv(a.K, 32) : cdiv(cdiv(a.K, 64), ksplit);
  const int ns = nk < 2 ? nk : 2;
  p.ns_flags = nk >= 2 ? ns | MVLT_NT_EARLY_DEFAULT : ns;
  long lds = (long)ns * (BM + bn) * (bk * 2);
  if (lds < stage) lds = stage;
  if (a.post_y) {
    MVLT_REQUIRE(epi == 2 && a.N == bn && a.a_map.mode == 0 && a.c_map.mode == 0 && a.c_map.rows_per_batch == 0 && a.post_gamma && a.post_beta &&
                 a.post_mean && a.post_rstd && a.post_ld % 8 == 0 && al16(a.post_y) && al16(a.post_gamma),
                 "mvlt_gemm_nt: post_y needs bf16 operands, a residual (R), N == 64 or 128, identity row maps, 16-byte aligned outputs");
    set_tp(p, MVLT_GEMM_NT_DMA, bn, 0, 8, 64);
    set_launch(p, gx, ksplit, 1, NTHREADS, lds < stage + 2048 ? stage + 2048 : lds);
    return MVLT_OK;
  }
  if (a.a_map.mode == 2 && (epi == 1 || epi == 2 || epi == 5) && a.split_k <= 1 && a.a_map.c_seg % 64 == 0 && a.c_map.mode == 0 &&
      (a.a_map.w_in == 16 || a.a_map.w_in == 32 || a.a_map.w_in == 64) && (a.a_map.h_in * a.a_map.w_in) % BM == 0 && a.M % BM == 0 &&
      a.M % (a.a_map.h_in * a.a_map.w_in) == 0 && a.a_map.hw_out == a.a_map.h_in * a.a_map.w_in && a.a_map.w_out == a.a_map.w_in &&
      a.K == 9 * a.a_map.c_seg && a.lda >= a.a_map.c_seg && a.ldb >= a.K) {
    const int w = a.a_map.w_in;
    const int cbn = (a.N % 192 == 0 && a.N % 128 != 0 && epi != 2) ? 192 : a.N <= 64 ? 64 : 128;
    const int halo_rows = (BM / w + 2) * (w + 2), h_it = cdiv(halo_rows * 8, NTHREADS);
    const long clds = (long)h_it * NTHREADS * 16 + (long)2 * cbn * ROW_BYTES, cstage = (long)4 * 32 * (cbn / 2 + 4) * sizeof(float);
    set_tp(p, MVLT_GEMM_NT_CONV3, w, cbn, epi);
    set_launch(p, 8 * cdiv(a.M / BM, 8) * cdiv(a.N, cbn), 1, 1, NTHREADS, clds < cstage ? cstage : clds);
    return MVLT_OK;
  }
  if (a.a_map.mode == 0 && a.a_map.rows_per_batch == 0 && a.c_map.mode == 0 && epi >= 1 && epi <= 5 && a.K % 64 == 0 && a.K >= 128) {
    auto cost = [&](int bm, int bnt) -> long {
      if (a.M % bm || a.N % bnt) return 0;
      const long tiles = (long)(a.M / bm) * (a.N / bnt);
      if (tiles < 192) return 0;
      return ((tiles + 255) / 256) * (long)bm * bnt;
    };
    auto mostly_real = [&](long tiles, double tile_elems) { return (double)a.M * a.N >= 0.85 * (double)((tiles + 255) / 256) * 256.0 * tile_elems; };
    const long c256 = cost(256, 256), c192 = cost(192, 256);
    const bool epi320 = a.N % 256 != 0 && (epi == 1 || (epi == 2 && a.K >= 640));
    const long c320 = epi320 ? cost(192, 320) : 0;
    if (!c320 && !c256 && !c192) {
      const long t256 = (long)cdiv(a.M, 256) * cdiv(a.N, 256);
      if (epi == 1 && (a.M % 256 || a.N % 256) && t256 >= 384 && mostly_real(t256, 65536.0)) { plan_nt_p8(a, p, 1, 4, 2, 2, 1); return MVLT_OK; }
      const long t320 = (long)cdiv(a.M, 192) * (a.N / 320);
      if (epi320 && a.N % 320 == 0 && a.M % 192 != 0 && t320 >= 192 && mostly_real(t320, 192.0 * 320.0)) { plan_nt_p8(a, p, epi, 3, 3, 2, 1); return MVLT_OK; }
    }
    if (c320) { plan_nt_p8(a, p, epi, 3, 3, 2, 0); return MVLT_OK; }
    if (c256 && (!c192 || c256 <= c192)) { plan_nt_p8(a, p, epi, 4, 2, 2, 0); return MVLT_OK; }
    if (c192) { plan_nt_p8(a, p, epi, 3, 2, 2, 0); return MVLT_OK; }
  }
  if (!narrow && a.N % 192 == 0 && a.N % 128 != 0 && (epi == 1 || epi == 5) && a.c_map.mode == 0 && a.a_map.mode != 1 && a.K >= 128) {
    const long lds192 = (long)ns * (BM + 192) * ROW_BYTES, stage192 = (long)4 * 32 * 100 * sizeof(float);
    set_tp(p, MVLT_GEMM_NT_DMA, 192, a.a_map.mode, epi, 64);
    set_launch(p, 8 * cdiv(tiles_m, 8) * (a.N / 192), 1, 1, NTHREADS, lds192 < stage192 ? stage192 : lds192);
    return MVLT_OK;
  }
  set_tp(p, MVLT_GEMM_NT_DMA, bn, a.a_map.mode, epi, bk);
  set_launch(p, gx, ksplit, 1, NTHREADS, lds);
  return MVLT_OK;
}

inline int plan_gemm_tn(const mvlt_gemm_tn_args& a, mvlt_gemm_plan& p) {
  using namespace mvlt_plan;
  p = mvlt_gemm_plan{};
  MVLT_REQUIRE(a.A && a.B && a.C, "mvlt_gemm_tn: null operand");
  MVLT_REQUIRE(a.M >= 0 && a.N1 > 0 && a.N2 > 0, "mvlt_gemm_tn: bad shape");
  MVLT_REQUIRE(a.dtype == 0 || a.dtype == 1, "mvlt_gemm_tn: dtype must be 0 (bf16) or 1 (fp32)");
  const int pc = a.dtype == 0 ? 8 : 4;
  MVLT_REQUIRE(a.lda % pc == 0 && a.ldb % pc == 0, "mvlt_gemm_tn: lda/ldb must be multiples of %d elements (16 B)", pc);
  MVLT_REQUIRE(a.lda >= (a.N1 + pc - 1) / pc * pc, "mvlt_gemm_tn: lda must cover N1 rounded up to %d", pc);
  MVLT_REQUIRE(a.b_map.mode != 0 || a.ldb >= (a.N2 + pc - 1) / pc * pc, "mvlt_gemm_tn: ldb must cover N2 rounded up to %d", pc);
  MVLT_REQUIRE(al16(a.A) && al16(a.B), "mvlt_gemm_tn: A/B must be 16-byte aligned");
  if (int e = check_rowmap(a.a_map, "mvlt_gemm_tn a_map")) return e;
  if (int e = check_rowmap(a.b_map, "mvlt_gemm_tn b_map")) return e;
  MVLT_REQUIRE(a.a_map.mode == 0, "mvlt_gemm_tn: A cannot be a patch gather");
  MVLT_REQUIRE(!(a.colsum_a && a.colsum_b), "mvlt_gemm_tn: at most one of colsum_a / colsum_b");
  MVLT_REQUIRE(a.b_map.mode == 0 || a.N2 == a.b_map.r * a.b_map.r * a.b_map.c_seg, "mvlt_gemm_tn: gather N2 != r*r*c_seg");
  MVLT_REQUIRE(a.c_taps <= 1 || (a.trans_c == 0 && a.c_seg > 0 && a.N2 == a.c_taps * a.c_seg), "mvlt_gemm_tn: c_taps needs trans_c == 0 and N2 == c_taps*c_seg");
  MVLT_REQUIRE(!a.dgrad_out || (a.dtype == 0 && a.M < (1 << 24) && a.b_map.mode == 0 && a.a_map.mode == 0),
               "mvlt_gemm_tn: dgrad_out rides on the bf16 LDS-DMA kernel only (bf16 operands, M < 2^24, plain row maps): every other path would leave it unwritten");
  if (a.M == 0) return MVLT_OK;
  const int mtiles = cdiv(a.M, TBK);
  constexpr int TN_MIN_TILES = 8;
  if (a.dtype == 0 && a.b_map.mode == 2 && a.a_map.mode == 0 && a.a_map.rows_per_batch == 0 && !a.trans_c && a.c_taps <= 1 &&
      !a.colsum_a && !a.colsum_b && a.N1 % 64 == 0 && a.b_map.c_seg % 64 == 0 && a.N2 == 9 * a.b_map.c_seg && a.M % 64 == 0 &&
      (a.b_map.w_in == 8 || a.b_map.w_in == 16 || a.b_map.w_in == 32 || a.b_map.w_in == 64) && (a.b_map.h_in * a.b_map.w_in) % 64 == 0 &&
      a.M % (a.b_map.h_in * a.b_map.w_in) == 0 && a.ldb >= a.b_map.c_seg) {
    const int w = a.b_map.w_in, halo_rows = (64 / w + 2) * (w + 2), h_it = cdiv(halo_rows * 8, NTHREADS);
    const long lds = (long)2 * (TN_TILE64_BYTES + h_it * NTHREADS * 16);
    const int n_o = a.N1 / 64, n_c = a.b_map.c_seg / 64;
    const Split sp = split_choose(cdiv(512, n_o * n_c), a.M / 64, 16, false);
    set_tp(p, MVLT_GEMM_TN_CONV3, w);
    set_launch(p, xcd_grid(sp.splits) * n_o * n_c, 1, 1, NTHREADS, lds);
    p.per_split = sp.per; p.t1 = n_o; p.t2 = n_c; p.splits = sp.splits;
    if (sp.splits >= 4 && a.ldc % 4 == 0 && al16(a.C) && lds >= (long)4 * 16 * (9 * 32 + 8) * 2 && scratch_fits(a, (long)sp.splits * a.N1 * a.N2 * 2)) plan_fold(a, p);
    return MVLT_OK;
  }
  if (a.partials && a.dtype == 0 && a.a_map.mode == 0 && a.b_map.mode == 0 && a.a_map.rows_per_batch == 0 && a.b_map.rows_per_batch == 0 && a.c_taps <= 1 &&
      !a.trans_c && !a.dgrad_out && a.M % 64 == 0 && a.ldc % 4 == 0 && al16(a.C) && al16(a.partials)) {
    const int nkt = a.M / 64;
    if (a.N1 % 256 == 0 && a.N2 % 256 == 0) {
      const int t1 = a.N1 / 256, t2 = a.N2 / 256, tiles = t1 * t2;
      if (tiles >= 16 && tiles <= 64 && nkt / (256 / tiles) >= 16 && a.partials_bytes >= (long)(256 / tiles) * a.N1 * a.N2 * 2) {
        const Split sp = split_even(256 / tiles, nkt);
        set_tp(p, MVLT_GEMM_TN_P8, 4, 2, 2, 1, 0, 0);
        set_launch(p, xcd_grid(sp.splits) * tiles, 1, 1, 512, 2 * 64 * 2 * (2 * (2 * 4 * 16) + 256));
        p.per_split = sp.per; p.t1 = t1; p.t2 = t2; p.splits = sp.splits;
        plan_fold(a, p);
        return MVLT_OK;
      }
    }
    const bool direct = a.N2 % 320 == 0 && a.N1 >= 1024, swapped = !direct && a.N1 % 320 == 0 && a.N2 >= 1024;
    if ((direct || swapped) && a.N1 % 8 == 0 && a.N2 % 8 == 0 && a.lda % 8 == 0 && a.ldb % 8 == 0) {
      const int rows = direct ? a.N1 : a.N2, cols = direct ? a.N2 : a.N1;
      const int t1 = cdiv(rows, 192), t2 = cols / 320, tiles = t1 * t2;
      if (tiles >= 6 && tiles <= 16 && nkt / (256 / tiles) >= 16 && (double)rows >= 0.85 * 192.0 * t1) {
        const Split sp = split_even((32 / tiles) * 8 >= 8 ? (32 / tiles) * 8 : 256 / tiles, nkt);
        if (scratch_fits(a, (long)sp.splits * a.N1 * a.N2 * 2)) {
          set_tp(p, MVLT_GEMM_TN_P8, 3, 3, 2, direct, rows % 192 != 0, swapped);
          set_launch(p, xcd_grid(sp.splits) * tiles, 1, 1, 512, 2 * 64 * 2 * (2 * (2 * 3 * 16) + 320));
          p.per_split = sp.per; p.t1 = t1; p.t2 = t2; p.splits = sp.splits; p.swap_operands = swapped;
          plan_fold(a, p);
          return MVLT_OK;
        }
      }
    }
  }
  if (a.dtype == 0 && a.M < (1 << 24)) {
    if (a.dgrad_out) {
      MVLT_REQUIRE(a.dgrad_wt && a.N1 == a.N2 && (a.N1 == 64 || a.N1 == 128) && a.a_map.rows_per_batch == 0 && a.b_map.mode == 0 &&
                   a.b_map.rows_per_batch == 0 && !a.trans_c && a.c_taps <= 1 && !a.colsum_b && a.dgrad_ld % 8 == 0 &&
                   (((uintptr_t)a.dgrad_out | (uintptr_t)a.dgrad_wt) & 15) == 0,
                   "mvlt_gemm_tn: dgrad_out needs bf16 operands, plain rows, N1 == N2 == 64 or 128, no transposed / tap output, 16-byte aligned buffers");
      const Split sp = split_choose(a.splits > 0 ? a.splits : (a.N1 == 64 ? 256 : 384), mtiles, TN_MIN_TILES, false);
      const int ns = a.N1 == 64 ? 4 : 2;
      set_tp(p, MVLT_GEMM_TN_DMA, a.N1, a.N1, 3, ns, 1);
      set_launch(p, xcd_grid(sp.splits), 1, 1, NTHREADS, (long)ns * TBK * 2 * a.N1 * 2 + 64 * a.N1 * 2);
      p.per_split = sp.per * TBK; p.t1 = 1; p.t2 = 1; p.splits = sp.splits;
      return MVLT_OK;
    }
    MVLT_REQUIRE(!a.c_overwrite || (!a.trans_c && a.c_taps <= 1 && a.N2 % 4 == 0 && a.ldc % 4 == 0 && al16(a.C)),
                 "mvlt_gemm_tn: c_overwrite needs the plain output layout, N2 % 4 == 0, ldc % 4 == 0 and a 16-byte aligned C");
    const bool small_out = a.N1 <= 128 && a.N2 <= 128;
    const int bmt = (a.N1 <= 64 || small_out) ? 64 : 128, bn = (a.N2 <= 64 || small_out) ? 64 : 128;
    const int t1 = cdiv(a.N1, bmt), t2 = cdiv(a.N2, bn);
    const int given = a.c_overwrite ? 1 : a.splits;
    const Split sp = given > 0 ? split_even(given, mtiles) : split_choose(cdiv(t1 * t2 == 1 ? 384 : 512, t1 * t2), mtiles, TN_MIN_TILES, true);
    const int ns = (bmt + bn == 256) ? 2 : (bmt + bn == 192) ? 3 : 4;
    const int bmode = (a.b_map.mode == 0 && a.b_map.rows_per_batch == 0 && a.a_map.rows_per_batch == 0) ? 3 : a.b_map.mode;
    set_tp(p, MVLT_GEMM_TN_DMA, bmt, bn, bmode, ns, 0);
    set_launch(p, xcd_grid(sp.splits) * t1 * t2, 1, 1, NTHREADS, (long)ns * TBK * (bmt + bn) * 2);
    p.per_split = sp.per * TBK; p.t1 = t1; p.t2 = t2; p.splits = sp.splits;
    constexpr int part_min = 8;
    constexpr long part_min_out = 16384;
    if (!a.c_overwrite && sp.splits >= part_min && !a.trans_c && a.c_taps <= 1 && a.N2 % 8 == 0 && a.ldc % 4 == 0 && al16(a.C) && (long)a.N1 * a.N2 >= part_min_out &&
        scratch_fits(a, (long)sp.splits * a.N1 * a.N2 * 2))
      plan_fold(a, p);
    return MVLT_OK;
  }
  const int bn = a.N2 <= 64 ? 64 : 128;
  const int t1 = cdiv(a.N1, BM), t2 = cdiv(a.N2, bn);
  const int want = cdiv(1024, t1 * t2);
  const Split sp = split_even(a.splits > 0 ? a.splits : (want > 4096 ? 4096 : want), mtiles);
  const int rowb = a.dtype == 0 ? TN_ROWB_BF16 : TN_ROWB_F32;
  set_tp(p, MVLT_GEMM_TN_PLAIN, a.dtype, bn);
  set_launch(p, t1, t2, sp.splits, NTHREADS, (long)(BM + bn) * rowb + BM * sizeof(float));
  p.per_split = sp.per * TBK; p.splits = sp.splits;
  return MVLT_OK;
}

inline int plan_kernel_name(const mvlt_gemm_plan& p, char* buf, size_t n) {
  const int* t = p.tp;
  const char* tf[2] = {"false", "true"};
  int w = -1;
  switch (p.family) {
    case MVLT_GEMM_NONE: w = snprintf(buf, n, "%s", ""); break;
    case MVLT_GEMM_NT_F32: w = snprintf(buf, n, "gemm_nt_kernel<float, %d>", t[0]); break;
    case MVLT_GEMM_NT_DMA: w = snprintf(buf, n, "gemm_nt_dma_kernel<%d, %d, %d, %d, 128>", t[0], t[1], t[2], t[3]); break;
    case MVLT_GEMM_NT_P8: w = snprintf(buf, n, "gemm_nt_p8_kernel<%d, %d, %d, %d, %s>", t[0], t[1], t[2], t[3], tf[t[4] != 0]); break;
    case MVLT_GEMM_NT_CONV3: w = snprintf(buf, n, "conv3_nt_kernel<%d, %d, %d>", t[0], t[1], t[2]); break;
    case MVLT_GEMM_TN_PLAIN:
      w = t[0] == 0 ? snprintf(buf, n, "_ZN12_GLOBAL__N_114gemm_tn_kernelIDF16bLi%dEEEv17mvlt_gemm_tn_argsi", t[1]) : snprintf(buf, n, "gemm_tn_kernel<float, %d>", t[1]);
      break;
    case MVLT_GEMM_TN_DMA: w = snprintf(buf, n, "gemm_tn_dma_kernel<%d, %d, %d, %d, %s>", t[0], t[1], t[2], t[3], tf[t[4] != 0]); break;
    case MVLT_GEMM_TN_P8: w = snprintf(buf, n, "gemm_tn_p8_kernel<%d, %d, %d, %s, %s, %s>", t[0], t[1], t[2], tf[t[3] != 0], tf[t[4] != 0], tf[t[5] != 0]); break;
    case MVLT_GEMM_TN_CONV3: w = snprintf(buf, n, "conv3_wgrad_kernel<%d>", t[0]); break;
    default: return -1;
  }
  return (w < 0 || (size_t)w >= n) ? -1 : w;
}
```

### mvlt_amd/heads.py

```python
import torch

from . import ops
from ._lib import rowmap
from .layers import StoreAccess, _empty, linear, linear_bwd
from .params import pool_zeros
from .plan import _EVERY, WORD_TABLE, plan_unit
from .pvlt import EPS_DEFAULT, VOCAB, VOCAB_LD


class _GradSink:

    def __init__(self, store):
        self.S, self.buf = store, None

    def take(self, shape, dtype, dev):
        if self.buf is None:
            self.buf = self.S.own(torch.zeros(shape, dtype=dtype, device=dev))
            return self.buf, self.buf
        return self.buf, None


def _embed_ln_fwd(model, prefix, A, a_map, rows):
    P, dt, dev = StoreAccess(model.store), model.compute_dtype, A.device
    Hd = model.hidden
    pre = _empty((rows, Hd), dt, dev)
    linear(A, P.w(prefix + ".0.weight"), pre, rows, a_map=a_map, bias=P.f32(prefix + ".0.bias"))
    y = _empty((rows, Hd), dt, dev)
    mean, rstd = _empty((rows,), torch.float32, dev), _empty((rows,), torch.float32, dev)
    ops.layernorm_fwd(pre, y, P.f32(prefix + ".1.weight"), P.f32(prefix + ".1.bias"), rows, Hd, Hd, Hd, EPS_DEFAULT, mean=mean, rstd=rstd)
    return y, (pre, mean, rstd)


def _embed_ln_bwd(model, prefix, dy, saved, A, a_map, rows, dA, c_map, accumulate, unit=_EVERY):
    P, dt, dev = StoreAccess(model.store), model.compute_dtype, dy.device
    Hd = model.hidden
    pre, mean, rstd = saved
    dpre = _empty((rows, Hd), dt, dev)
    ops.layernorm_bwd(dy, pre, dpre, P.f32(prefix + ".1.weight"), mean, rstd, rows, Hd, Hd, Hd, Hd,
                      dgamma=P.g(prefix + ".1.weight"), dbeta=P.g(prefix + ".1.bias"))
    linear_bwd(unit.launches["embed"], dpre, A, P.g(prefix + ".0.weight"), P.g(prefix + ".0.bias"), P.wT(prefix + ".0.weight"), dA, rows,
               x_map=a_map, dx_map=c_map, R=dA if accumulate else None)


class _ClsHeadFn(torch.autograd.Function):

    @staticmethod
    def forward(ctx, x4, model, name, HW, sink):
        P, dt, dev = StoreAccess(model.store), model.compute_dtype, x4.device
        B, N, C = x4.shape
        n_out = P.f32(name + "_head.linear.weight").shape[0]
        a_map = rowmap(1, N, HW)
        e, saved = _embed_ln_fwd(model, name + "_head_embed", x4, a_map, B)
        bias = (P.f32(name + "_head.linear.bias") + P.f32(name + "_head.linear_bias")).contiguous()
        logits = _empty((B, n_out), torch.float32, dev)
        linear(e, P.w(name + "_head.linear.weight"), logits, bias=bias)
        ctx.pack = (model, name, HW, x4, e, saved, a_map, sink)
        ctx.unit = plan_unit(model, name + "_head")
        return logits.view(B, 1, n_out)

    @staticmethod
    def backward(ctx, dlogits):
        model, name, HW, x4, e, saved, a_map, sink = ctx.pack
        S, dt, dev, P = model.store, model.compute_dtype, x4.device, StoreAccess(model.store)
        S.queue_finalize()
        u = ctx.unit
        B, N, C = x4.shape
        n_out = dlogits.shape[-1]
        n_pad = (n_out + 7) // 8 * 8
        dl = _empty((B, n_pad), dt, dev)
        if n_pad <= 256:
            ops.head_grad_prep(dlogits.reshape(B, n_out).float().contiguous(), dl, P.g(name + "_head.linear.bias"), P.g(name + "_head.linear_bias"))
        else:
            dl.zero_()
            dl[:, :n_out] = dlogits.reshape(B, n_out).to(dt)
            db = dlogits.reshape(B, n_out).float().sum(0)
            P.g(name + "_head.linear.bias").add_(db)
            P.g(name + "_head.linear_bias").add_(db)
        de = _empty((B, model.hidden), dt, dev)
        linear_bwd(u.launches["linear"], dl, e, P.g(name + "_head.linear.weight"), None, P.wT(name + "_head.linear.weight"), de)
        dx4, ret = (sink or _GradSink(S)).take(x4.shape, dt, dev) if u.dgrad else (None, None)
        _embed_ln_bwd(model, name + "_head_embed", de, saved, x4, a_map, B, dx4, a_map, True, u)
        ctx.pack = ctx.unit = None
        S.announce_prefix(name + "_head_embed.", name + "_head.")
        return ret, None, None, None, None


def _mlm_transform_fwd(model, rows_in, R):
    P, dt, dev = StoreAccess(model.store), model.compute_dtype, rows_in.device
    Hd = model.hidden
    hp, ga = _empty((R, Hd), dt, dev), _empty((R, Hd), dt, dev)
    linear(rows_in, P.w("mlm_head.transform.dense.weight"), ga, bias=P.f32("mlm_head.transform.dense.bias"), act=1, H=hp)
    t = _empty((R, Hd), dt, dev)
    mean, rstd = _empty((R,), torch.float32, dev), _empty((R,), torch.float32, dev)
    ops.layernorm_fwd(ga, t, P.f32("mlm_head.transform.LayerNorm.weight"), P.f32("mlm_head.transform.LayerNorm.bias"),
                      R, Hd, Hd, Hd, EPS_DEFAULT, mean=mean, rstd=rstd)
    return t, (hp, ga, mean, rstd)


def _mlm_transform_bwd(model, dt_, saved, rows_in, R, unit=_EVERY):
    P, dt, dev = StoreAccess(model.store), model.compute_dtype, dt_.device
    Hd = model.hidden
    hp, ga, mean, rstd = saved
    dga = _empty((R, Hd), dt, dev)
    ops.layernorm_bwd(dt_, ga, dga, P.f32("mlm_head.transform.LayerNorm.weight"), mean, rstd, R, Hd, Hd, Hd, Hd,
                      dgamma=P.g("mlm_head.transform.LayerNorm.weight"), dbeta=P.g("mlm_head.transform.LayerNorm.bias"))
    dhp = ops.gelu_bwd(dga, hp, torch.empty_like(dga))
    din = _empty((R, Hd), dt, dev)
    linear_bwd(unit.launches["dense"], dhp, rows_in, P.g("mlm_head.transform.dense.weight"), P.g("mlm_head.transform.dense.bias"),
               P.wT("mlm_head.transform.dense.weight"), din)
    return din


class _MLMFullFn(torch.autograd.Function):

    @staticmethod
    def forward(ctx, x4, model, HW, sink):
        P, dt, dev = StoreAccess(model.store), model.compute_dtype, x4.device
        B, N, C = x4.shape
        T = N - HW
        R = B * T
        a_map = rowmap(T, N, HW)
        e, sv_e = _embed_ln_fwd(model, "mlm_head_embed", x4, a_map, R)
        t, sv_t = _mlm_transform_fwd(model, e, R)
        buf = _empty((R, VOCAB_LD), torch.float32, dev)
        linear(t, P.w(WORD_TABLE), buf, bias=P.f32("mlm_head.bias"))
        ctx.pack = (model, HW, x4, e, sv_e, t, sv_t, a_map, sink)
        ctx.unit = plan_unit(model, "mlm_head")
        return buf.view(B, T, VOCAB_LD)[:, :, :VOCAB]

    @staticmethod
    def backward(ctx, dlogits):
        model, HW, x4, e, sv_e, t, sv_t, a_map, sink = ctx.pack
        S, dt, dev = model.store, model.compute_dtype, x4.device
        S.queue_finalize()
        B, N, C = x4.shape
        T = N - HW
        R = B * T
        dl = torch.zeros(R, VOCAB_LD, device=dev, dtype=dt)
        dl[:, :VOCAB] = dlogits.reshape(R, VOCAB).to(dt)
        u = ctx.unit
        dx4, ret = (sink or _GradSink(S)).take(x4.shape, dt, dev) if u.dgrad else (None, None)
        _mlm_decoder_bwd(model, dl, t, sv_t, e, sv_e, x4, a_map, R, dx4, accumulate=True, unit=u)
        ctx.pack = ctx.unit = None
        return ret, None, None, None


def _mlm_decoder_bwd(model, dl, t, sv_t, e, sv_e, A, a_map, R, dA, c_map=None, accumulate=False, unit=_EVERY):
    S, dt, dev, P = model.store, model.compute_dtype, dl.device, StoreAccess(model.store)
    Hd = model.hidden
    if unit.launches["table"]:
        linear_bwd(True, dl, t, P.g(WORD_TABLE), P.g("mlm_head.bias"),
                   overwrite=dt == torch.bfloat16 and S.all_zeroed_this_pass and WORD_TABLE not in S.touched_this_pass)
        S.touched_this_pass.add(WORD_TABLE)
    elif unit.launches["bias"]:
        db = _empty((1, VOCAB_LD), torch.float32, dev)
        ops.batch_sum(dl, db, R, 1, VOCAB_LD, 1, VOCAB_LD)
        P.g("mlm_head.bias").add_(db[0, :VOCAB])
    wT = P.wT(WORD_TABLE)
    if dt == torch.bfloat16:
        dtr32 = pool_zeros((R, Hd), torch.float32, dev)
        linear(dl, wT, dtr32, split_k=4)
        dtr = dtr32.to(dt)
    else:
        dtr = _empty((R, Hd), dt, dev)
        linear(dl, wT, dtr)
    de = _mlm_transform_bwd(model, dtr, sv_t, e, R, unit)
    _embed_ln_bwd(model, "mlm_head_embed", de, sv_e, A, a_map, R, dA, c_map if c_map is not None else a_map, accumulate, unit)
    S.announce_prefix("mlm_head_embed.", "mlm_head.")


class _MLMFusedFn(torch.autograd.Function):

    @staticmethod
    def forward(ctx, x4, model, HW, positions, labels_sel, sink):
        P, dt, dev = StoreAccess(model.store), model.compute_dtype, x4.device
        B, N, C = x4.shape
        T = N - HW
        R = positions.numel()
        rows = _empty((R, C), dt, dev)
        tmap = rowmap(T, N, HW)
        ops.gather_rows(x4, positions, rows, R, C, C, src_map=tmap)
        e, sv_e = _embed_ln_fwd(model, "mlm_head_embed", rows, None, R)
        t, sv_t = _mlm_transform_fwd(model, e, R)
        logits = _empty((R, VOCAB_LD), torch.float32, dev)
        linear(t, P.w(WORD_TABLE), logits, bias=P.f32("mlm_head.bias"))
        lse = _empty((R,), torch.float32, dev)
        ctx.smoothing = smoothing = model.loss_options.mlm_label_smoothing
        if smoothing:
            acc = _empty((3,), torch.float32, dev)
            ops.ce_smooth_fwd(logits, labels_sel, lse, _empty((R,), torch.float32, dev), acc, R, VOCAB, VOCAB_LD, label_smoothing=smoothing)
        else:
            acc = pool_zeros((2,), torch.float32, dev)
            ops.cross_entropy_fwd(logits, labels_sel, lse, acc[0:1], acc[1:2], R, VOCAB, VOCAB_LD)
        ctx.pack = (model, HW, x4.shape, rows, e, sv_e, t, sv_t, logits, lse, acc, positions, labels_sel, tmap, sink)
        ctx.unit = plan_unit(model, "mlm_head")
        return acc[0] / acc[1]

    @staticmethod
    def backward(ctx, gloss):
        model, HW, xshape, rows, e, sv_e, t, sv_t, logits, lse, acc, positions, labels_sel, tmap, sink = ctx.pack
        S, dt, dev = model.store, model.compute_dtype, rows.device
        S.queue_finalize()
        B, N, C = xshape
        R = positions.numel()
        dl = _empty((R, VOCAB_LD), dt, dev)
        gs = gloss.reshape(1).float().contiguous()
        if ctx.smoothing:
            ops.ce_smooth_bwd(logits, labels_sel, lse, gs, acc, dl, R, VOCAB, VOCAB_LD, VOCAB_LD, label_smoothing=ctx.smoothing)
        else:
            ops.cross_entropy_bwd(logits, labels_sel, lse, gs, acc[1:2], dl, R, VOCAB, VOCAB_LD, VOCAB_LD)
        u = ctx.unit
        drows = _empty((R, C), dt, dev) if u.dgrad else None
        _mlm_decoder_bwd(model, dl, t, sv_t, e, sv_e, rows, None, R, drows, c_map=None, unit=u)
        ret = None
        if u.dgrad:
            dx4, ret = (sink or _GradSink(S)).take(xshape, dt, dev)
            ops.scatter_rows(drows, positions, dx4, R, C, C, dst_map=tmap, accumulate=True)
        ctx.pack = ctx.unit = None
        return ret, None, None, None, None, None
```

### mvlt_amd/layers.py

```python
import torch

from . import ops


def _empty(shape, dtype, dev):
    return torch.empty(shape, dtype=dtype, device=dev)


class StoreAccess:

    def __init__(self, S):
        self.S = S

    def w(self, name):
        return self.S.comp(name)

    def wT(self, name):
        return self.S.extra[name + "::T"]

    def wK(self, name):
        return self.S.extra[name + "::K"]

    def wKT(self, name):
        return self.S.extra[name + "::KT"]

    def f32(self, name):
        return self.S.master(name)

    def g(self, name):
        return self.S.grad(name)

    def gl(self, name):
        return self.S.grad_copies(name)

    def lnk(self):
        return self.S.ln_kwargs()


def _rows(t):
    return t.numel() // t.shape[-1]


def linear(x, W, y, M=None, **epi):
    N = W.shape[0]
    K = W.numel() // N
    return ops.gemm_nt(x, W, y, _rows(x) if M is None else M, N, K, x.stride(-2), K, y.stride(-2), **epi)


def linear_bwd(on, dy, x, gW, gb, wT=None, dx=None, M=None, *, fuse=False, tn=None, dy_map=None, x_map=None, dx_map=None, overwrite=False, **epi):
    if on:
        rows, N1 = _rows(dy) if M is None else M, gW.shape[0]
        N2 = gW.numel() // N1
        if fuse:
            return ops.gemm_tn(dy, x, gW, rows, N1, N2, dy.stride(-2), x.stride(-2), N2, colsum=gb, dgrad=(wT, dx))
        ops.gemm_tn(dy, x, gW, rows, N1, N2, dy.stride(-2), x.stride(-2), N2, a_map=dy_map, b_map=x_map, colsum=gb,
                    partials=None if tn is None else tn.tn_partials(), defer_fold=tn is not None, overwrite=overwrite)
    if dx is not None:
        linear(dy, wT, dx, M, a_map=dy_map, c_map=dx_map, **epi)


def conv_wgrad(S, name, dz, xin, bmap, colsum=None):
    cout, taps, cin = dz.shape[-1], bmap.r * bmap.r, bmap.c_seg
    ops.gemm_tn(dz, xin, S.grad_taps(name, cout, taps, cin), _rows(dz), cout, taps * cin, dz.stride(-2), xin.stride(-2), taps * cin, b_map=bmap, colsum=colsum,
                partials=S.tn_partials(), defer_fold=True)
```

### mvlt_amd/ops.py

```python
import ctypes as C

import torch

from . import _lib as L
from ._lib import DT, check, patchmap, ptr, rowmap, stream_ptr

_ID = rowmap()


def _gemm_nt_args(A, B, C_out, M, N, K, lda, ldb, ldc, *, a_map=None, c_map=None, bias=None, act=0, H=None,
                  row_scale=None, rows_per_scale=0, R=None, col_sum=None, col_sumsq=None, col_copies=0, split_k=0, post_ln=None):
    assert A.dtype == B.dtype and A.dtype in DT and (C_out.dtype in DT or (C_out.dtype == torch.float16 and col_sum is not None))
    if bias is not None:
        assert bias.dtype == torch.float32
    if row_scale is not None:
        assert row_scale.dtype == torch.float32
    if R is not None:
        assert R.dtype == C_out.dtype or (R.dtype == torch.float32 and C_out.dtype == torch.bfloat16)
    if H is not None:
        assert H.dtype == C_out.dtype
    if col_sum is not None:
        assert col_sum.dtype == torch.float32 and col_sumsq is not None and col_sumsq.dtype == torch.float32
    a = L.GemmNTArgs(A=ptr(A), B=ptr(B), C=ptr(C_out), M=M, N=N, K=K, lda=lda, ldb=ldb, ldc=ldc,
                     dtype=DT[A.dtype], out_dtype=2 if C_out.dtype == torch.float16 else DT[C_out.dtype], a_map=a_map or _ID, c_map=c_map or _ID,
                     bias=ptr(bias), act=act, H=ptr(H), row_scale=ptr(row_scale), rows_per_scale=rows_per_scale, R=ptr(R),
                     col_sum=ptr(col_sum), col_sumsq=ptr(col_sumsq), col_copies=col_copies, split_k=split_k)
    if R is not None and R.dtype != C_out.dtype:
        a.r_fp32 = 1
    if post_ln is not None:
        g, b, eps, y, mean, rstd = post_ln
        assert g.dtype == b.dtype == mean.dtype == rstd.dtype == torch.float32 and y.dtype == torch.bfloat16 and y.is_contiguous()
        a.post_y, a.post_ld, a.post_gamma, a.post_beta, a.post_eps, a.post_mean, a.post_rstd = ptr(y), y.shape[-1], ptr(g), ptr(b), eps, ptr(mean), ptr(rstd)
    return a


def gemm_nt(A, B, C_out, *dims, **kw):
    check(L.lib.mvlt_gemm_nt(C.byref(_gemm_nt_args(A, B, C_out, *dims, **kw)), stream_ptr()), "mvlt_gemm_nt")
    return C_out


class Plan:

    def __init__(self, plan_fn, args, cls=None, name_fn=None):
        p, buf = (cls or L.GemmPlan)(), C.create_string_buffer(256)
        check(plan_fn(C.byref(args), C.byref(p)), "plan")
        check(min((name_fn or L.lib.mvlt_gemm_plan_name)(C.byref(p), buf, len(buf)), 0), "plan name")
        self.p, self.name = p, buf.value.decode()

    def __getattr__(self, field):
        v = getattr(self.p, field)
        return v if isinstance(v, int) else list(v)


def gemm_nt_plan(*args, **kw):
    return Plan(L.lib.mvlt_gemm_nt_plan, _gemm_nt_args(*args, **kw))


def gemm_tn_plan(*args, **kw):
    return Plan(L.lib.mvlt_gemm_tn_plan, _gemm_tn_args(*args, **kw))


def tn_fold_flush(partials=None):
    check(L.lib.mvlt_tn_fold_flush(ptr(partials), stream_ptr()), "mvlt_tn_fold_flush")


def tn_fold_discard(partials=None):
    check(L.lib.mvlt_tn_fold_discard(ptr(partials)), "mvlt_tn_fold_discard")


def weight_prep(desc_dev, blk_dev, ndesc, total_blocks, dtype, blk_desc=None):
    check(L.lib.mvlt_weight_prep(ptr(desc_dev), ptr(blk_dev), ndesc, total_blocks, ptr(blk_desc), DT[dtype], stream_ptr()), "mvlt_weight_prep")


def gemm_tn(A, B, C_out, *dims, **kw):
    check(L.lib.mvlt_gemm_tn(C.byref(_gemm_tn_args(A, B, C_out, *dims, **kw)), stream_ptr()), "mvlt_gemm_tn")
    return C_out


def _gemm_tn_args(A, B, C_out, M, N1, N2, lda, ldb, ldc, *, a_map=None, b_map=None, colsum=None, splits=0, taps=0, seg=0, dgrad=None, partials=None, defer_fold=False, overwrite=False):
    assert A.dtype == B.dtype and A.dtype in DT and C_out.dtype == torch.float32
    if colsum is not None:
        assert colsum.dtype == torch.float32
    a_map, b_map = a_map or _ID, b_map or _ID
    swap = dgrad is None and N1 <= 64 < N2 and b_map.mode == 0 and taps <= 1 and partials is None
    if swap:
        A, B, N1, N2, lda, ldb, a_map, b_map = B, A, N2, N1, ldb, lda, b_map, a_map
    a = L.GemmTNArgs(A=ptr(A), B=ptr(B), C=ptr(C_out), M=M, N1=N1, N2=N2, lda=lda, ldb=ldb, ldc=ldc, dtype=DT[A.dtype], a_map=a_map, b_map=b_map, splits=splits)
    if swap:
        a.colsum_b, a.trans_c = ptr(colsum), 1
    elif dgrad is not None:
        wt, dx = dgrad
        assert A.dtype == torch.bfloat16 and wt.dtype == dx.dtype == torch.bfloat16 and N1 == N2 and N1 in (64, 128) and taps <= 1
        assert wt.is_contiguous() and tuple(wt.shape) == (N2, N1) and dx.stride(-1) == 1
        dgrad_ld = dx.stride(-2) if dx.dim() >= 2 else N2
        assert dgrad_ld % 8 == 0 and dgrad_ld >= N2, dgrad_ld
        assert a_map.mode == 0 and a_map.rows_per_batch == 0 and b_map.mode == 0 and b_map.rows_per_batch == 0, "gemm_tn(dgrad=...): plain row maps only"
        a.colsum_a, a.dgrad_wt, a.dgrad_out, a.dgrad_ld = ptr(colsum), ptr(wt), ptr(dx), dgrad_ld
    else:
        a.colsum_a, a.c_taps, a.c_seg = ptr(colsum), taps, seg
        if partials is not None:
            a.partials, a.partials_bytes = ptr(partials), partials.numel() * partials.element_size()
            a.defer_fold = 1 if defer_fold else 0
    if overwrite and dgrad is None:
        assert not a.trans_c and taps <= 1 and N2 % 4 == 0 and ldc % 4 == 0 and A.dtype == torch.bfloat16, "gemm_tn(overwrite=True): bf16, plain output layout, N2 and ldc multiples of 4"
        a.c_overwrite = 1
    return a


LN_CHAIN_WIDTHS = (64, 128, 320, 512, 768)


def layernorm_fwd(x, y, gamma, beta, rows, Cdim, ldx, ldy, eps, *, mean=None, rstd=None, add=None, add_rows=0,
                  x_map=None, y_map=None, chain=None):
    assert x.dtype in DT and y.dtype in DT and gamma.dtype == torch.float32 and beta.dtype == torch.float32
    a = L.LayerNormArgs(x=ptr(x), y=ptr(y), gamma=ptr(gamma), beta=ptr(beta), mean=ptr(mean), rstd=ptr(rstd), add=ptr(add), add_rows=add_rows,
                        rows=rows, C=Cdim, ldx=ldx, ldy=ldy, x_map=x_map or _ID, y_map=y_map or _ID, eps=eps, dtype=DT[x.dtype], y_dtype=DT[y.dtype])
    if chain is not None:
        g2, b2, eps2, y2, m2, r2 = chain
        assert Cdim in LN_CHAIN_WIDTHS and y2.dtype == torch.bfloat16 and g2.dtype == b2.dtype == m2.dtype == r2.dtype == torch.float32
        a.y2, a.gamma2, a.beta2, a.eps2, a.mean2, a.rstd2 = ptr(y2), ptr(g2), ptr(b2), eps2, ptr(m2), ptr(r2)
    check(L.lib.mvlt_layernorm_fwd(C.byref(a), stream_ptr()), "mvlt_layernorm_fwd")
    return y


def layernorm_bwd(dy, x, dx, gamma, mean, rstd, rows, Cdim, lddy, ldx, lddx, *, dgamma=None, dbeta=None,
                  dy_map=None, x_map=None, dx_map=None, accumulate=False, dx2=None, dx2_scale=None, dx2_rows_per_scale=0, lddx2=0,
                  copies=1, copy_stride=0):
    assert dy.dtype in DT and x.dtype in DT and dx.dtype in DT
    assert dx2 is None or (dx2.dtype == dy.dtype and dx2_scale is not None and dx2_scale.dtype == torch.float32 and dx2_rows_per_scale > 0)
    a = L.LayerNormBwdArgs(dy=ptr(dy), x=ptr(x), dx=ptr(dx), gamma=ptr(gamma), mean=ptr(mean), rstd=ptr(rstd), dgamma=ptr(dgamma), dbeta=ptr(dbeta),
                           rows=rows, C=Cdim, lddy=lddy, ldx=ldx, lddx=lddx, dy_map=dy_map or _ID, x_map=x_map or _ID, dx_map=dx_map or _ID,
                           dx_accumulate=1 if accumulate else 0, dtype=DT[dy.dtype], x_dtype=DT[x.dtype], dx_dtype=DT[dx.dtype],
                           dx2=ptr(dx2), dx2_scale=ptr(dx2_scale), dx2_rows_per_scale=dx2_rows_per_scale, lddx2=lddx2, dg_copies=copies, dg_copy_stride=copy_stride)
    check(L.lib.mvlt_layernorm_bwd(C.byref(a), stream_ptr()), "mvlt_layernorm_bwd")
    return dx


def fold_copies(arena, copies, stride, dst_index, j0, j1, dst):
    assert arena.dtype == torch.float32 and dst.dtype == torch.float32 and dst_index.dtype == torch.int32
    check(L.lib.mvlt_fold_copies(ptr(arena), copies, stride, ptr(dst_index), j0, j1, ptr(dst), stream_ptr()), "mvlt_fold_copies")


def batch_sum(x, out, B, R, Cdim, batch_stride_rows, ld, acc2=None, split=0):
    assert out.dtype == torch.float32 and (acc2 is None or (acc2.dtype == torch.float32 and acc2.is_contiguous()))
    check(L.lib.mvlt_batch_sum(ptr(x), ptr(out), B, R, Cdim, batch_stride_rows, ld, DT[x.dtype], ptr(acc2), split, stream_ptr()), "mvlt_batch_sum")
    return out


def _attention_fwd_args(Q, KV, O, lse, B, H, N, M, ldq, ldkv, ldo, k_off, v_off, scale):
    assert Q.dtype == KV.dtype == O.dtype and Q.dtype in DT
    return L.AttnArgs(Q=ptr(Q), KV=ptr(KV), O=ptr(O), lse=ptr(lse), B=B, H=H, N=N, M=M, ldq=ldq, ldkv=ldkv, ldo=ldo, k_off=k_off, v_off=v_off,
                      scale=scale, dtype=DT[Q.dtype])


def _attention_bwd_args(Q, KV, O, dO, lse, dQ, dKV, B, H, N, M, ldq, ldkv, ldo, lddkv, k_off, v_off, scale):
    assert dKV.dtype == torch.float32 or (dKV.dtype == torch.bfloat16 and Q.dtype == torch.bfloat16)
    return L.AttnBwdArgs(Q=ptr(Q), KV=ptr(KV), O=ptr(O), dO=ptr(dO), lse=ptr(lse), dQ=ptr(dQ), dKV=ptr(dKV), B=B, H=H, N=N, M=M,
                         ldq=ldq, ldkv=ldkv, ldo=ldo, lddkv=lddkv, k_off=k_off, v_off=v_off, scale=scale, dtype=DT[Q.dtype], dkv_dtype=DT[dKV.dtype])


def _attention_fwd(entry, *args):
    check(getattr(L.lib, entry)(C.byref(_attention_fwd_args(*args)), stream_ptr()), entry)
    return args[2]


def _attention_bwd(entry, *args):
    check(getattr(L.lib, entry)(C.byref(_attention_bwd_args(*args)), stream_ptr()), entry)
    return args[5], args[6]


def attention_plan(*args, streamed=False):
    fwd = len(args) == 14
    a = (_attention_fwd_args if fwd else _attention_bwd_args)(*args)
    plan_fn = L.lib.mvlt_sr_attention_fwd_plan if fwd else L.lib.mvlt_sr_attention_bwd_plan
    return Plan(lambda args_ref, plan_ref: plan_fn(args_ref, int(streamed), plan_ref), a, L.AttnPlan, L.lib.mvlt_attn_plan_name)


def sr_attention_fwd(Q, KV, O, lse, B, H, N, M, ldq, ldkv, ldo, k_off, v_off, scale):
    return _attention_fwd("mvlt_sr_attention_fwd", Q, KV, O, lse, B, H, N, M, ldq, ldkv, ldo, k_off, v_off, scale)


def sr_attention_bwd_chunks(B, H, N, M, dtype):
    return int(L.lib.mvlt_sr_attention_bwd_chunks(B, H, N, M, DT[dtype]))


def sr_attention_bwd(Q, KV, O, dO, lse, dQ, dKV, B, H, N, M, ldq, ldkv, ldo, lddkv, k_off, v_off, scale):
    return _attention_bwd("mvlt_sr_attention_bwd", Q, KV, O, dO, lse, dQ, dKV, B, H, N, M, ldq, ldkv, ldo, lddkv, k_off, v_off, scale)


def sr_attention_fwd_streamed(Q, KV, O, lse, B, H, N, M, ldq, ldkv, ldo, k_off, v_off, scale):
    return _attention_fwd("mvlt_sr_attention_fwd_streamed", Q, KV, O, lse, B, H, N, M, ldq, ldkv, ldo, k_off, v_off, scale)


def sr_attention_bwd_streamed(Q, KV, O, dO, lse, dQ, dKV, B, H, N, M, ldq, ldkv, ldo, lddkv, k_off, v_off, scale):
    return _attention_bwd("mvlt_sr_attention_bwd_streamed", Q, KV, O, dO, lse, dQ, dKV, B, H, N, M, ldq, ldkv, ldo, lddkv, k_off, v_off, scale)


def bert_embed_fwd(ids, word, pos, type0, gamma, beta, keep, drop_p, y, mean, rstd, rows, T, eps):
    assert ids.dtype == torch.int64 and (keep is None or keep.dtype == torch.uint8)
    check(L.lib.mvlt_bert_embed_fwd(ptr(ids), ptr(word), ptr(pos), ptr(type0), ptr(gamma), ptr(beta), ptr(keep), drop_p,
                                    ptr(y), ptr(mean), ptr(rstd), rows, T, word.shape[1], eps, DT[y.dtype], stream_ptr()),
          "mvlt_bert_embed_fwd")
    return y


def bert_embed_bwd(dy, ids, word, pos, type0, gamma, keep, drop_p, mean, rstd, dword, dpos, dtype0, dgamma, dbeta, rows, T):
    check(L.lib.mvlt_bert_embed_bwd(ptr(dy), ptr(ids), ptr(word), ptr(pos), ptr(type0), ptr(gamma), ptr(keep), drop_p,
                                    ptr(mean), ptr(rstd), ptr(dword), ptr(dpos), ptr(dtype0), ptr(dgamma), ptr(dbeta),
                                    rows, T, word.shape[1], DT[dy.dtype], stream_ptr()), "mvlt_bert_embed_bwd")


def head_grad_prep(dlogits, dl, db1, db2=None):
    assert dlogits.dtype == torch.float32 and dlogits.is_contiguous() and dl.is_contiguous() and dl.dtype in DT and db1.dtype == torch.float32
    B, n = dlogits.shape
    check(L.lib.mvlt_head_grad_prep(ptr(dlogits), B, n, dl.shape[1], ptr(dl), ptr(db1), ptr(db2), DT[dl.dtype], stream_ptr()), "mvlt_head_grad_prep")


def patchify(img, out, B, Cin, H, W, k):
    assert img.dtype == torch.float32 and img.is_contiguous()
    check(L.lib.mvlt_patchify(ptr(img), ptr(out), B, Cin, H, W, k, DT[out.dtype], stream_ptr()), "mvlt_patchify")
    return out


def masked_select(labels, idx, count, ignore_index=-1):
    assert labels.dtype == torch.int64 and idx.dtype == torch.int32 and count.dtype == torch.int32 and labels.is_contiguous()
    check(L.lib.mvlt_masked_select(ptr(labels), labels.numel(), ignore_index, ptr(idx), ptr(count), stream_ptr()), "mvlt_masked_select")


def gather_rows(src, idx, dst, rows, Cdim, ld_src, src_map=None):
    assert idx.dtype == torch.int32 and src.dtype == dst.dtype
    m = C.byref(src_map) if src_map is not None else None
    check(L.lib.mvlt_gather_rows(ptr(src), ptr(idx), ptr(dst), rows, Cdim, ld_src, m, DT[src.dtype], stream_ptr()), "mvlt_gather_rows")
    return dst


def scatter_rows(src, idx, dst, rows, Cdim, ld_dst, dst_map=None, accumulate=False):
    assert idx.dtype == torch.int32 and src.dtype == dst.dtype
    m = C.byref(dst_map) if dst_map is not None else None
    check(L.lib.mvlt_scatter_rows(ptr(src), ptr(idx), ptr(dst), rows, Cdim, ld_dst, m, 1 if accumulate else 0, DT[src.dtype], stream_ptr()),
          "mvlt_scatter_rows")
    return dst


def cross_entropy_fwd(logits, labels, lse, loss_sum, count, rows, V, ld, ignore_index=-1):
    assert labels.dtype == torch.int64
    check(L.lib.mvlt_cross_entropy_fwd(ptr(logits), ptr(labels), ignore_index, ptr(lse), ptr(loss_sum), ptr(count), rows, V, ld,
                                       DT[logits.dtype], stream_ptr()), "mvlt_cross_entropy_fwd")


def cross_entropy_bwd(logits, labels, lse, gscale, count, dlogits, rows, V, ld, ldd, ignore_index=-1):
    check(L.lib.mvlt_cross_entropy_bwd(ptr(logits), ptr(labels), ignore_index, ptr(lse), ptr(gscale), ptr(count), ptr(dlogits), rows, V, ld, ldd,
                                       DT[logits.dtype], DT[dlogits.dtype], stream_ptr()), "mvlt_cross_entropy_bwd")


def _ce_smooth_ok(logits, labels, weight, rows, V, ld, label_smoothing):
    assert logits.dtype in DT and logits.is_contiguous() and labels.dtype == torch.int64 and labels.is_contiguous()
    assert labels.numel() >= rows and (rows <= 0 or logits.numel() >= (rows - 1) * ld + V)
    assert weight is None or (weight.dtype == torch.float32 and weight.is_contiguous() and weight.numel() >= V)
    return float(label_smoothing)


def ce_smooth_fwd(logits, labels, lse, smooth, acc, rows, V, ld, *, ignore_index=-1, label_smoothing=0.0, weight=None):
    e = _ce_smooth_ok(logits, labels, weight, rows, V, ld, label_smoothing)
    for t, n in ((lse, rows), (smooth, rows), (acc, 3)):
        assert t.dtype == torch.float32 and t.is_contiguous() and t.numel() >= n
    check(L.lib.mvlt_ce_smooth_fwd(ptr(logits), ptr(labels), ignore_index, e, ptr(weight), ptr(lse), ptr(smooth), ptr(acc), rows, V, ld, DT[logits.dtype],
                                   stream_ptr()), "mvlt_ce_smooth_fwd")


def ce_smooth_bwd(logits, labels, lse, gscale, acc, dlogits, rows, V, ld, ldd, *, ignore_index=-1, label_smoothing=0.0, weight=None):
    e = _ce_smooth_ok(logits, labels, weight, rows, V, ld, label_smoothing)
    for t, n in ((lse, rows), (gscale, 1), (acc, 3)):
        assert t.dtype == torch.float32 and t.is_contiguous() and t.numel() >= n
    assert dlogits.dtype in DT and dlogits.is_contiguous() and (rows <= 0 or dlogits.numel() >= rows * ldd)
    check(L.lib.mvlt_ce_smooth_bwd(ptr(logits), ptr(labels), ignore_index, e, ptr(weight), ptr(lse), ptr(gscale), ptr(acc), ptr(dlogits), rows, V, ld, ldd,
                                   DT[logits.dtype], DT[dlogits.dtype], stream_ptr()), "mvlt_ce_smooth_bwd")


ADAMW_FROZEN = 2


def adamw_step(p, g, m, v, p16, n, hp, decay_mask=None, *, gscale_dev=None):
    assert decay_mask is None or decay_mask.dtype == torch.uint8
    if gscale_dev is not None:
        assert gscale_dev.dtype == torch.float32
    check(L.lib.mvlt_adamw_step(ptr(p), ptr(g), ptr(m), ptr(v), ptr(p16), n, ptr(hp), ptr(decay_mask), ptr(gscale_dev), stream_ptr()), "mvlt_adamw_step")


def grad_sumsq(g, n, mask, partials):
    assert g.dtype == torch.float32 and partials.dtype == torch.float32 and g.is_contiguous() and partials.is_contiguous()
    assert g.numel() >= n and (mask is None or (mask.dtype == torch.uint8 and mask.is_cuda and mask.is_contiguous() and mask.numel() >= n))
    check(L.lib.mvlt_grad_sumsq(ptr(g), n, ptr(mask), ptr(partials), partials.numel(), stream_ptr()), "mvlt_grad_sumsq")


def clip_coef(partials, grad_scale, max_norm, out):
    assert partials.dtype == torch.float32 and out.dtype == torch.float32 and out.numel() >= 2 and out.is_contiguous() and partials.is_contiguous()
    check(L.lib.mvlt_clip_coef(ptr(partials), partials.numel(), float(grad_scale), float(max_norm), ptr(out), stream_ptr()), "mvlt_clip_coef")


def step_gate(partials, grad_scale, max_norm, out, counters):
    assert partials.dtype == torch.float32 and out.dtype == torch.float32 and out.numel() >= 4 and out.is_contiguous() and partials.is_contiguous()
    assert counters.dtype == torch.int32 and counters.numel() >= 2 and counters.is_contiguous()
    check(L.lib.mvlt_step_gate(ptr(partials), partials.numel(), float(grad_scale), float(max_norm), ptr(out), ptr(counters), stream_ptr()), "mvlt_step_gate")


def adamw_step_gated(p, g, m, v, p16, n, hp, decay_mask, gate):
    assert decay_mask is None or decay_mask.dtype == torch.uint8
    assert gate.dtype == torch.float32 and gate.numel() >= 4 and gate.is_contiguous()
    check(L.lib.mvlt_adamw_step_gated(ptr(p), ptr(g), ptr(m), ptr(v), ptr(p16), n, ptr(hp), ptr(decay_mask), ptr(gate), stream_ptr()), "mvlt_adamw_step_gated")


OPT_FROZEN = 255
OPT_MAX_GROUPS = 254


def adamw_step_groups(p, g, m, v, p16, n, hp, group_of, table, n_groups, *, gscale_dev=None, gate=None):
    for t in (p, g, m, v, hp, table):
        assert t.dtype == torch.float32 and t.is_contiguous()
    assert min(p.numel(), g.numel(), m.numel(), v.numel(), group_of.numel()) >= n and hp.numel() >= 8 and table.numel() >= 2 * n_groups
    assert p16 is None or (p16.dtype == torch.bfloat16 and p16.is_contiguous() and p16.numel() >= n)
    assert group_of.dtype == torch.uint8 and group_of.is_contiguous()
    assert gscale_dev is None or gscale_dev.dtype == torch.float32
    assert gate is None or (gate.dtype == torch.float32 and gate.numel() >= 4 and gate.is_contiguous())
    check(L.lib.mvlt_adamw_step_groups(ptr(p), ptr(g), ptr(m), ptr(v), ptr(p16), n, ptr(hp), ptr(group_of), ptr(table), n_groups, ptr(gscale_dev), ptr(gate),
                                       stream_ptr()), "mvlt_adamw_step_groups")


LAMB_CHUNK = 16384
LAMB_ROW = 6
LAMB_ALWAYS_ADAPT = 1
LAMB_TRUST_CLIP = 2


def lamb_check_tables(tensors, chunks, n, n_groups):
    assert tensors.dtype == torch.int64 and chunks.dtype == torch.int32 and not tensors.is_cuda and not chunks.is_cuda
    assert tensors.is_contiguous() and chunks.is_contiguous() and tensors.numel() % LAMB_ROW == 0 and chunks.numel() % 2 == 0
    check(L.lib.mvlt_lamb_check_tables(tensors.data_ptr() or None, tensors.numel() // LAMB_ROW, chunks.data_ptr() or None, chunks.numel() // 2, n, n_groups),
          "mvlt_lamb_check_tables")


def _lamb_tables_ok(tensors, chunks):
    assert tensors.dtype == torch.int64 and tensors.is_contiguous() and tensors.numel() % LAMB_ROW == 0
    assert chunks.dtype == torch.int32 and chunks.is_contiguous() and chunks.numel() % 2 == 0
    return tensors.numel() // LAMB_ROW, chunks.numel() // 2


def lamb_moments(p, g, m, v, n, hp, tensors, chunks, table, n_groups, partials, *, gscale_dev=None, gate=None):
    nt, nc = _lamb_tables_ok(tensors, chunks)
    for t in (p, g, m, v, hp, table, partials):
        assert t.dtype == torch.float32 and t.is_contiguous()
    assert min(p.numel(), g.numel(), m.numel(), v.numel()) >= n and hp.numel() >= 8 and table.numel() >= 2 * n_groups and partials.numel() >= 2 * nc
    assert gscale_dev is None or gscale_dev.dtype == torch.float32
    assert gate is None or (gate.dtype == torch.float32 and gate.numel() >= 4 and gate.is_contiguous())
    check(L.lib.mvlt_lamb_moments(ptr(p), ptr(g), ptr(m), ptr(v), n, ptr(hp), ptr(tensors), nt, ptr(chunks), nc, ptr(table), n_groups, ptr(partials),
                                  ptr(gscale_dev), ptr(gate), stream_ptr()), "mvlt_lamb_moments")


def lamb_fold(partials, tensors, n_chunks, table, n_groups, flags, ratios, *, gate=None):
# ... 335 lines not shown
```

### mvlt_amd/params.py

```python
import math
import weakref
from collections import OrderedDict

import torch
import torch.nn as nn

from . import ops

_TN_SCRATCH_MIB = 256
ALIGN = 8


class Holder(nn.Module):

    def __init__(self, **shapes):
        super().__init__()
        for name, shape in shapes.items():
            self.register_parameter(name, nn.Parameter(torch.zeros(*shape)))


def affine(n):
    return Holder(weight=(n,), bias=(n,))


def linear(n_out, n_in, bias=True):
    return Holder(weight=(n_out, n_in), bias=(n_out,)) if bias else Holder(weight=(n_out, n_in))


def trunc_normal_(t, std=0.02):
    return nn.init.trunc_normal_(t, mean=0.0, std=std, a=-2.0, b=2.0)


def conv_default_init_(w, b):
    nn.init.kaiming_uniform_(w, a=math.sqrt(5))
    if b is not None:
        fan_in = w[0].numel()
        bound = 1 / math.sqrt(fan_in)
        nn.init.uniform_(b, -bound, bound)


def prep_blocks(d):
    if d.kind == 1:
        return (d.d0 * d.d1 * d.d2 + 255) // 256
    return ((d.R + 63) // 64) * ((d.C + 63) // 64)


def pack_prep_table(descs, dtype, device):
    import ctypes
    from ._lib import MVLTError, PrepDesc
    blocks = []
    for i, d in enumerate(descs):
        if d.kind not in (0, 1, 2):
            raise MVLTError(f"weight_prep descriptor {i}: kind {d.kind} is not 0 (transpose), 1 (gather) or 2 (bf16 transpose)")
        if d.kind == 2 and dtype != torch.bfloat16:
            raise MVLTError(f"weight_prep descriptor {i}: kind 2 (transpose of a bf16 source) needs a bf16 destination, the table is {dtype}")
        if d.kind == 2 and (d.C % 8 or d.ld_out % 8):
            raise MVLTError(f"weight_prep descriptor {i}: kind 2 needs C and ld_out in multiples of 8, got C {d.C}, ld_out {d.ld_out}")
        if d.kind != 1 and d.ld_out < d.R:
            raise MVLTError(f"weight_prep descriptor {i}: ld_out {d.ld_out} < R {d.R}")
        b = prep_blocks(d)
        if b < 1:
            raise MVLTError(f"weight_prep descriptor {i}: empty")
        blocks.append(b)
    arr = (PrepDesc * len(descs))(*descs)
    raw = torch.frombuffer(bytearray(ctypes.string_at(ctypes.addressof(arr), ctypes.sizeof(arr))), dtype=torch.uint8)
    starts = [0]
    for b in blocks:
        starts.append(starts[-1] + b)
    blk = torch.tensor(starts, dtype=torch.int32, device=device)
    blk_desc = torch.repeat_interleave(torch.arange(len(blocks), dtype=torch.int32), torch.tensor(blocks)).to(torch.int32).to(device)
    return raw.to(device), blk, len(descs), starts[-1], blk_desc


class ZeroPool:
    _pools = {}

    class Token:
        __slots__ = ("__weakref__",)

    def __init__(self, device):
        self.device, self.buf, self.used, self.need = device, None, 0, 0
        self._live = weakref.WeakSet()

    @classmethod
    def of(cls, device):
        key = (device.type, device.index)
        if key not in cls._pools:
            cls._pools[key] = cls(device)
        return cls._pools[key]

    @property
    def pending(self):
        return len(self._live)

    def reset(self, grad_on=False):
        want = max(self.need, self.used)
        if self.pending > 0:
            self.buf = None
        tok = None
        if grad_on:
            tok = ZeroPool.Token()
            self._live.add(tok)
        if self.buf is None or want > self.buf.numel():
            self.buf = torch.empty(int(want * 1.25) + (1 << 20), dtype=torch.uint8, device=self.device)
            want = self.buf.numel()
        if want:
            self.buf[:want].zero_()
        self.used, self.need = 0, 0
        return tok

    def take(self, shape, dtype):
        n = 1
        for d in shape:
            n *= int(d)
        nbytes = (n * torch.empty((), dtype=dtype).element_size() + 255) // 256 * 256
        self.need += nbytes
        if self.buf is None or self.used + nbytes > self.buf.numel():
            return torch.zeros(shape, dtype=dtype, device=self.device)
        t = self.buf[self.used:self.used + nbytes].view(dtype)[:n].view(shape)
        self.used += nbytes
        return t


def pool_zeros(shape, dtype, device):
    return ZeroPool.of(torch.device(device) if not isinstance(device, torch.device) else device).take(tuple(shape) if not isinstance(shape, int) else (shape,), dtype)


class FlatStore:

    def __init__(self, module, compute_dtype):
        self.module = module
        self.compute_dtype = compute_dtype
        self.device = None
        self.P = self.G = self.C = None
        self._views = {}
        self.offsets = OrderedDict()
        self.params = OrderedDict()
        self._module_slots, self._param_slots = [], []
        self.total = 0
        self._cast_version = -1
        self.refresh_count = 0
        self._c_fresh_version = None
        self.extra = {}
        self._finalize_queued = False
        self.force_dirty = True
        self.fn_params = []
        self.on_backward_done = None
        self.on_range_ready = None
        self.on_pass_aborted = None
        self._ranges_done = []
        self.all_zeroed_this_pass = False
        self.touched_this_pass = set()
        self.scale_in_optimizer = False
        self.pending_grad_scale = 1.0
        self.pending_clip = None
        self._clip = None
        self.pending_gate = None
        self._gate = None
        self.grad_works = []

    def _index(self):
        self.offsets.clear()
        self.params.clear()
        off = 0
        seen = set()
        for name, p in self.module.named_parameters():
            if id(p) in seen:
                continue
            seen.add(id(p))
            n = p.numel()
            self.offsets[name] = (off, n, tuple(p.shape))
            self.params[name] = p
            off += (n + ALIGN - 1) // ALIGN * ALIGN
        self.total = off
        self.fn_params = list(self.params.items())
        self._module_slots = [(m._modules, k, c) for m in self.module.modules() for k, c in m._modules.items() if c is not None]
        off_of = {id(p): self.offsets[name][0] for name, p in self.params.items()}
        self._param_slots = [(m._parameters, k, p, off_of[id(p)]) for m in self.module.modules() for k, p in m._parameters.items() if p is not None]

    def is_current(self):
        if self.P is None:
            return False
        for d, k, c in self._module_slots:
            if d.get(k) is not c:
                return False
        base = self.P.data_ptr()
        for d, k, p, off in self._param_slots:
            q = d.get(k)
            if q is not p or q.data_ptr() != base + 4 * off:
                return False
        return True

    def materialize(self, device):
        self._index()
        P = torch.zeros(self.total, device=device, dtype=torch.float32)
        for name, p in self.params.items():
            off, n, shape = self.offsets[name]
            P[off:off + n].copy_(p.detach().reshape(-1).to(device=device, dtype=torch.float32))
        self.P = P
        self.G = torch.zeros_like(P)
        for name, p in self.params.items():
            off, n, shape = self.offsets[name]
            p.data = P[off:off + n].view(shape)
            p.grad = None
        self.C = torch.empty(self.total, device=device, dtype=torch.bfloat16) if self.compute_dtype == torch.bfloat16 else None
        self.device = device
        self.extra = {}
        self._cast_version = -1
        self._c_fresh_version = None
        self._plist = list(self.params.values())
        self.force_dirty = True

    def ensure(self, device):
        if self.device != device or not self.is_current():
            self.materialize(device)

    def _view(self, kind, buf, name):
        cache = self._views.get(kind)
        if cache is None or cache[0] is not buf:
            cache = self._views[kind] = (buf, {})
        v = cache[1].get(name)
        if v is None:
            off, n, shape = self.offsets[name]
            v = cache[1][name] = buf[off:off + n].view(shape)
        return v

    def master(self, name):
        return self._view("P", self.P, name)

    def grad(self, name):
        off, n, shape = self.offsets[name]
        return self.G[off:off + n].view(shape)

    def comp(self, name):
        return self._view("C", self.C if self.C is not None else self.P, name)

    def versions(self):
        return self.P._version + sum(p._version for p in self._plist)

    def invalidate(self):
        self.force_dirty = True
        self._c_fresh_version = None
        self._cast_version = -1

    def c_is_current(self):
        return self.C is not None and self.versions() in (self._cast_version, self._c_fresh_version)

    def c_written_by_kernel(self, was_current, wrote_all):
        self.force_dirty = True
        self._c_fresh_version = self.versions() if self.C is not None and (wrote_all or was_current) else None

    def refresh(self, transposed, conv_perm, conv3=()):
        ver = self.versions()
        if not self.force_dirty and self._cast_version == ver:
            return
        if self.C is not None and self._c_fresh_version != ver:
            ops.cast_bf16(self.P, self.C, self.total)
        self._c_fresh_version = None
        key = (tuple(transposed), tuple(conv_perm), tuple(conv3), self.compute_dtype, self.P.data_ptr())
        if getattr(self, "_prep_key", None) != key:
            self._build_prep(transposed, conv_perm, conv3)
            self._prep_key = key
        if self._prep_n:
            ops.weight_prep(self._prep_desc, self._prep_blk, self._prep_n, self._prep_blocks, self.compute_dtype, self._prep_blk_desc)
        self._cast_version = ver
        self.force_dirty = False
        self.refresh_count += 1

    def _build_prep(self, transposed, conv_perm, conv3):
        from ._lib import PrepDesc
        dt, dev = self.compute_dtype, self.device
        descs, blocks = [], []

        def src_ptr(name):
            return self.master(name).data_ptr()

        def transpose(name):
            w = self.master(name)
            R, Ccols = w.shape
            ld = (R + 7) // 8 * 8
            k = name + "::T"
            if k not in self.extra or self.extra[k].dtype != dt or self.extra[k].device != dev:
                self.extra[k] = torch.zeros(Ccols, ld, device=dev, dtype=dt)
            if self.C is not None and dt == torch.bfloat16 and Ccols % 8 == 0:
                descs.append(PrepDesc(self.comp(name).data_ptr(), self.extra[k].data_ptr(), 2, R, Ccols, ld, 0, 0, 0, 0, 0, 0, 0, 0, 0, 0))
            else:
                descs.append(PrepDesc(src_ptr(name), self.extra[k].data_ptr(), 0, R, Ccols, ld, 0, 0, 0, 0, 0, 0, 0, 0, 0, 0))
            blocks.append(((R + 63) // 64) * ((Ccols + 63) // 64))

        def gather(name, suffix, shape, dims, src_off, ss, ds):
            k = name + suffix
            if k not in self.extra or self.extra[k].dtype != dt or tuple(self.extra[k].shape) != tuple(shape) or self.extra[k].device != dev:
                self.extra[k] = torch.zeros(*shape, device=dev, dtype=dt)
            descs.append(PrepDesc(src_ptr(name), self.extra[k].data_ptr(), 1, 0, 0, 0, dims[0], dims[1], dims[2], src_off,
                                  ss[0], ss[1], ss[2], ds[0], ds[1], ds[2]))
            blocks.append((dims[0] * dims[1] * dims[2] + 255) // 256)

        for name in transposed:
            transpose(name)
        for name in list(conv_perm) + list(conv3):
            out, cin, kh, kw = self.master(name).shape
            t = kh * kw
            gather(name, "::K", (out, t * cin), (out, t, cin), 0, (cin * t, 1, t), (t * cin, cin, 1))
            if name in conv_perm:
                gather(name, "::KT", (t * cin, out), (t, cin, out), 0, (1, t, cin * t), (cin * out, out, 1))
            else:
                gather(name, "::F", (cin, t * out), (cin, t, out), t - 1, (t, -1, cin * t), (t * out, out, 1))
        if "t2i_head.score.0.weight" in self.offsets and conv3:
            name = "t2i_head.score.0.weight"
            K = self.master(name).numel() // 3
            gather(name, "::W", (3, K), (1, 1, 3 * K), 0, (0, 0, 1), (0, 0, 1))
            gather(name, "::T", (K, 8), (K, 3, 1), 0, (1, K, 0), (8, 1, 0))
        self._prep_n = len(descs)
        if not descs:
            return
        assert blocks == [prep_blocks(d) for d in descs]
        self._prep_desc, self._prep_blk, self._prep_n, self._prep_blocks, self._prep_blk_desc = pack_prep_table(descs, dt, dev)

    def begin_backward(self):
        self.wait_grads()
        if self.G.is_cuda:
            from . import ops
            if getattr(self, "_tn_partials", None) is not None:
                ops.tn_fold_discard(self._tn_partials)
        live = [(n, q) for n, q in self.fn_params if q.requires_grad]
        alias = [q.grad is not None and q.grad.data_ptr() == self.grad(n).data_ptr() for n, q in live]
        self.all_zeroed_this_pass = not any(alias)
        self.touched_this_pass = set()
        if not any(alias):
            self.G.zero_()
            self.pending_grad_scale = 1.0
            self.pending_clip = None
            self.pending_gate = None
        else:
            self.apply_pending_scale()
            runs = []
            for (n, _), a in zip(live, alias):
                if a:
                    continue
                off, cnt, _ = self.offsets[n]
                hi = off + (cnt + ALIGN - 1) // ALIGN * ALIGN
                if runs and runs[-1][1] == off:
                    runs[-1][1] = hi
                else:
                    runs.append([off, hi])
            for lo, hi in runs:
                self.G[lo:hi].zero_()
        self._ranges_done = []
        self._own = set()
        if getattr(self, "_tap_lo", None) is not None:
            self._tap_arena.zero_()
            self._tap_lo = self._tap_hi = None
        if getattr(self, "_ln_lo", None) is not None:
            self._ln_arena[:, self._ln_lo:self._ln_hi].zero_()
            self._ln_lo = self._ln_hi = None

    def own(self, t):
        self._own.add(t.data_ptr())
        return t

    def owns(self, t):
        return t is not None and t.data_ptr() in getattr(self, "_own", ())

    def new_pass(self):
        if self._finalize_queued:
            self._finalize_queued = False
            self._ranges_done = []
            if self.on_pass_aborted is not None:
                self.on_pass_aborted(self)

    def queue_finalize(self):
        if self._finalize_queued:
            return
        self._finalize_queued = True
        self.begin_backward()
        torch.autograd.Variable._execution_engine.queue_callback(self._finalize)

    def _finalize(self):
        self._finalize_queued = False
        self.fold_copies()
        if self.on_backward_done is not None:
            self.on_backward_done(self)

    def stage_range(self, i):
        names = [n for n in self.offsets if n.startswith((f"patch_embed{i+1}.", f"text_embed{i+1}.", f"block{i+1}."))]
        lo = self.offsets[names[0]][0]
        o, n, _ = self.offsets[names[-1]]
        return lo, o + (n + ALIGN - 1) // ALIGN * ALIGN

    LN_COPIES = 256

    @property
    def ln_stride(self):
        if getattr(self, "_ln_stride", None) is None:
            total = sum(n for _, n, shape in self.offsets.values() if len(shape) == 1)
            self._ln_stride = (total + 63) // 64 * 64
        return self._ln_stride

    def ln_kwargs(self):
        return dict(copies=self.LN_COPIES, copy_stride=self.ln_stride)

    def grad_copies(self, name):
        if getattr(self, "_ln_arena", None) is None or self._ln_arena.device != self.G.device:
            self._ln_arena = torch.zeros(self.LN_COPIES, self.ln_stride, device=self.G.device, dtype=torch.float32)
            self._ln_index = torch.zeros(self.ln_stride, device=self.G.device, dtype=torch.int32)
            self._ln_slots, self._ln_next, self._ln_lo, self._ln_hi = {}, 0, None, None
        goff, n, _ = self.offsets[name]
        slot = self._ln_slots.get(name)
        if slot is None:
            assert self._ln_next + n <= self.ln_stride, "LayerNorm gradient arena too small"
            slot = self._ln_slots[name] = self._ln_next
            self._ln_index[slot:slot + n] = torch.arange(goff, goff + n, device=self.G.device, dtype=torch.int32)
            self._ln_next += n
        self._ln_lo = slot if self._ln_lo is None else min(self._ln_lo, slot)
        self._ln_hi = slot + n if self._ln_hi is None else max(self._ln_hi, slot + n)
        return self._ln_arena[0, slot:slot + n]

    def fold_copies(self, early=False):
        from . import ops
        if early and self.on_range_ready is None:
            return
        if self.G.is_cuda:
            self.tn_fold_flush()
        if getattr(self, "_tap_lo", None) is not None:
            ops.fold_copies(self._tap_arena, 1, self._tap_arena.numel(), self._tap_index, self._tap_lo, self._tap_hi, self.G)
            self._tap_lo = self._tap_hi = None
        if getattr(self, "_ln_lo", None) is None:
            return
        ops.fold_copies(self._ln_arena, self.LN_COPIES, self.ln_stride, self._ln_index, self._ln_lo, self._ln_hi, self.G)
        self._ln_lo = self._ln_hi = None

    def grad_taps(self, name, cout, taps, cin):
        if getattr(self, "_tap_arena", None) is None or self._tap_arena.device != self.G.device:
            total = sum(n for _, n, shape in self.offsets.values() if len(shape) == 4)
            self._tap_arena = torch.zeros((total + 63) // 64 * 64, device=self.G.device, dtype=torch.float32)
            self._tap_index = torch.zeros(self._tap_arena.numel(), device=self.G.device, dtype=torch.int32)
            self._tap_slots, self._tap_next, self._tap_lo, self._tap_hi = {}, 0, None, None
        goff, n, _ = self.offsets[name]
        assert n == cout * taps * cin, (name, n, cout, taps, cin)
        slot = self._tap_slots.get(name)
        if slot is None:
            slot = self._tap_slots[name] = self._tap_next
            dev = self.G.device
            o = torch.arange(cout, device=dev, dtype=torch.int64)[:, None, None]
            t = torch.arange(taps, device=dev, dtype=torch.int64)[None, :, None]
            c = torch.arange(cin, device=dev, dtype=torch.int64)[None, None, :]
            self._tap_index[slot:slot + n] = (goff + (o * cin + c) * taps + t).reshape(-1).to(torch.int32)
            self._tap_next += n
        self._tap_lo = slot if self._tap_lo is None else min(self._tap_lo, slot)
        self._tap_hi = slot + n if self._tap_hi is None else max(self._tap_hi, slot + n)
        return self._tap_arena[slot:slot + n].view(cout, taps * cin)

    def announce_stage(self, i):
        self.fold_copies(early=True)
        if self.on_range_ready is not None:
            lo, hi = self.stage_range(i)
            self._ranges_done.append((lo, hi))
            self.on_range_ready(self, lo, hi)

    def prefix_range(self, prefixes):
        names = [n for n in self.offsets if n.startswith(prefixes)]
        if not names:
            return None
        lo = self.offsets[names[0]][0]
        o, n, _ = self.offsets[names[-1]]
        hi = o + (n + ALIGN - 1) // ALIGN * ALIGN
        assert sum((self.offsets[k][1] + ALIGN - 1) // ALIGN * ALIGN for k in names) == hi - lo, ("not contiguous", prefixes)
        return lo, hi

    def announce_prefix(self, *prefixes):
        if self.on_range_ready is None:
            return
        r = self.prefix_range(tuple(prefixes))
        if r is not None:
            if self.G.is_cuda:
                self.tn_fold_flush()
            self._ranges_done.append(r)
            self.on_range_ready(self, *r)

    def scale_grads(self, factor):
        if self.scale_in_optimizer:
            self.pending_grad_scale *= factor
        else:
            self.G.mul_(factor)

    def tn_fold_flush(self):
        if getattr(self, "_tn_partials", None) is not None:
            from . import ops
            ops.tn_fold_flush(self._tn_partials)

    def tn_partials(self):
        t = getattr(self, "_tn_partials", None)
        if t is None or t.device != self.G.device:
            t = self._tn_partials = torch.empty(_TN_SCRATCH_MIB * 8 * 65536, dtype=torch.bfloat16, device=self.G.device)
        return t

    def wait_grads(self):
        works, self.grad_works = self.grad_works, []
        for w, lo, hi, g, t, early in works:
            w.wait()
            if t is not None:
                g.copy_(t)

    def apply_pending_scale(self):
        self.wait_grads()
        if self.pending_grad_scale != 1.0:
            self.G.mul_(self.pending_grad_scale)
            self.pending_grad_scale = 1.0
        if self.pending_clip is not None:
            clip, self.pending_clip = self.pending_clip, None
            ops.scale_by_dev(self.G, self.total, clip)
        if self.pending_gate is not None:
            gate, self.pending_gate = self.pending_gate, None
            ops.scale_by_dev(self.G, self.total, gate[1:2])

    CLIP_PARTIALS = 1024

    def _clip_buffers(self):
        key = (self.G.data_ptr(), tuple(p.requires_grad for p in self._plist))
        if self._clip is None or self._clip[0] != key:
            mask = torch.zeros(self.total, dtype=torch.uint8)
            for name, p in self.params.items():
                if p.requires_grad:
                    off, n, _ = self.offsets[name]
                    mask[off:off + n] = 1
            dev = self.G.device
            old = self._clip
            part = old[2] if old is not None and old[2].device == dev else torch.empty(self.CLIP_PARTIALS, device=dev, dtype=torch.float32)
            out = old[3] if old is not None and old[3].device == dev else torch.zeros(2, device=dev, dtype=torch.float32)
            self._clip = (key, mask.to(dev), part, out)
        return self._clip[1:]

    @torch.no_grad()
    def clip_grad_norm(self, max_norm):
        self.wait_grads()
        self.sync_grads()
        if self.pending_clip is not None or self.pending_gate is not None:
            self.apply_pending_scale()
        mask, part, out = self._clip_buffers()
        ops.grad_sumsq(self.G, self.total, mask, part)
        ops.clip_coef(part, self.pending_grad_scale, max_norm, out)
        self.pending_clip = out[1:2]
        return out[0]

    def _gate_buffers(self):
        dev = self.G.device
        if self._gate is None:
            self._gate = (torch.zeros(4, device=dev, dtype=torch.float32), torch.zeros(2, device=dev, dtype=torch.int32))
        elif self._gate[0].device != dev:
            self._gate = (self._gate[0].to(dev), self._gate[1].to(dev))
        return self._gate

    @torch.no_grad()
    def gate_grads(self, max_norm=None):
        self.wait_grads()
        self.sync_grads()
        if self.pending_clip is not None or self.pending_gate is not None:
            self.apply_pending_scale()
        mask, part, _ = self._clip_buffers()
        out, counters = self._gate_buffers()
        ops.grad_sumsq(self.G, self.total, mask, part)
        ops.step_gate(part, self.pending_grad_scale, max_norm or 0.0, out, counters)
        self.pending_gate = out
        return out[0]

    def sync_grads(self):
        for name, p in self.params.items():
            gv = self.grad(name)
            if p.grad is None:
                continue
            if p.grad.data_ptr() != gv.data_ptr():
                gv.copy_(p.grad)
                p.grad = gv
```

Baseline: 13100.

## Add NN GEMM reading untransposed weights for MLM head input gradient

Adds an NN-form GEMM variant of the DMA NT kernel that loads B with k-major rows and builds its fragments with a transposed LDS read. The MLM head's input gradient now multiplies directly by the word-embedding table instead of a transposed copy. The per-step transpose of the word-embedding weight in the prep pass is skipped. This removes the transpose kernel's work and the memory for the transposed copy, at the cost of a new kernel path whose LDS fragment reads may be slower than the NT layout.

```diff
diff --git a/include/mvlt_hip_nn.h b/include/mvlt_hip_nn.h
--- /dev/null
+++ b/include/mvlt_hip_nn.h
@@ -0,0 +1,24 @@
+#ifndef MVLT_HIP_NN_H
+#define MVLT_HIP_NN_H
+#include "mvlt_hip.h"
+#include "mvlt_hip_plan.h"
+#ifdef __cplusplus
+extern "C" {
+#endif
+
+#define MVLT_NN_VERSION 1
+int mvlt_nn_version(void);
+
+typedef struct mvlt_gemm_nn_args {
+  mvlt_gemm_nt_args nt;
+  int b_rows;
+} mvlt_gemm_nn_args;
+
+int mvlt_gemm_nn(const mvlt_gemm_nn_args* args, void* stream);
+int mvlt_gemm_nn_plan(const mvlt_gemm_nn_args* args, mvlt_gemm_plan* plan);
+int mvlt_gemm_nn_sizeof(void);
+
+#ifdef __cplusplus
+}
+#endif
+#endif
diff --git a/mvlt_amd/_lib.py b/mvlt_amd/_lib.py
--- a/mvlt_amd/_lib.py
+++ b/mvlt_amd/_lib.py
@@ -317,6 +317,28 @@
 if lib.mvlt_ingest_version() != INGEST_VERSION:
     raise ImportError(f"ingest entry points mismatch: {LIB_PATH} is version {lib.mvlt_ingest_version()}, the binding is version {INGEST_VERSION} (stale build? run python -m mvlt_amd.build)")
 
+class GemmNNArgs(C.Structure):
+    _fields_ = [("nt", GemmNTArgs), ("b_rows", c_int)]
+
+
+NN_STRUCTS = (("mvlt_gemm_nn_args", GemmNNArgs),)
+NN_PROTOTYPES = {
+    "mvlt_nn_version": (_i, []),
+    "mvlt_gemm_nn": _by_args(GemmNNArgs),
+    "mvlt_gemm_nn_plan": (_i, [C.POINTER(GemmNNArgs), C.POINTER(GemmPlan)]),
+    "mvlt_gemm_nn_sizeof": (_i, []),
+}
+for _name, (_res, _args) in NN_PROTOTYPES.items():
+    if not hasattr(lib, _name):
+        raise ImportError(f"{LIB_PATH} does not export {_name} (include/mvlt_hip_nn.h): stale build? run python -m mvlt_amd.build")
+    _fn = getattr(lib, _name)
+    _fn.restype, _fn.argtypes = _res, _args
+
+NN_VERSION = 1
+if lib.mvlt_nn_version() != NN_VERSION or lib.mvlt_gemm_nn_sizeof() != C.sizeof(GemmNNArgs):
+    raise ImportError(f"NN GEMM entry points mismatch: {LIB_PATH} is version {lib.mvlt_nn_version()} with {lib.mvlt_gemm_nn_sizeof()} bytes of mvlt_gemm_nn_args, the binding is "
+                      f"version {NN_VERSION} with {C.sizeof(GemmNNArgs)} (stale build? run python -m mvlt_amd.build)")
+
 DT = {torch.bfloat16: 0, torch.float32: 1}
 
 
diff --git a/mvlt_amd/build.py b/mvlt_amd/build.py
--- a/mvlt_amd/build.py
+++ b/mvlt_amd/build.py
@@ -20,7 +20,7 @@
     import hashlib
     h = hashlib.sha256()
     files = sorted(os.path.join(CSRC, f) for f in os.listdir(CSRC) if f.endswith((".hip", ".h", ".inc")))
-    files += [os.path.join(HERE, "..", "include", h) for h in ("mvlt_hip.h", "mvlt_hip_ext.h", "mvlt_hip_ema.h", "mvlt_hip_plan.h", "mvlt_hip_opt.h", "mvlt_hip_lamb.h", "mvlt_hip_loss.h", "mvlt_hip_ingest.h")]
+    files += [os.path.join(HERE, "..", "include", h) for h in ("mvlt_hip.h", "mvlt_hip_ext.h", "mvlt_hip_ema.h", "mvlt_hip_plan.h", "mvlt_hip_opt.h", "mvlt_hip_lamb.h", "mvlt_hip_loss.h", "mvlt_hip_ingest.h", "mvlt_hip_nn.h")]
     for f in files:
         h.update(os.path.basename(f).encode())
         h.update(open(f, "rb").read())
@@ -29,7 +29,7 @@
 
 def _deps_mtime():
     hdrs = [os.path.join(CSRC, f) for f in os.listdir(CSRC) if f.endswith((".h", ".inc"))]
-    hdrs += [os.path.join(HERE, "..", "include", h) for h in ("mvlt_hip.h", "mvlt_hip_ext.h", "mvlt_hip_ema.h", "mvlt_hip_plan.h", "mvlt_hip_opt.h", "mvlt_hip_lamb.h", "mvlt_hip_loss.h", "mvlt_hip_ingest.h")]
+    hdrs += [os.path.join(HERE, "..", "include", h) for h in ("mvlt_hip.h", "mvlt_hip_ext.h", "mvlt_hip_ema.h", "mvlt_hip_plan.h", "mvlt_hip_opt.h", "mvlt_hip_lamb.h", "mvlt_hip_loss.h", "mvlt_hip_ingest.h", "mvlt_hip_nn.h")]
     return max(os.path.getmtime(h) for h in hdrs)
 
 
diff --git a/mvlt_amd/csrc/gemm.hip b/mvlt_amd/csrc/gemm.hip
--- a/mvlt_amd/csrc/gemm.hip
+++ b/mvlt_amd/csrc/gemm.hip
@@ -152,6 +152,19 @@
   return p.family == MVLT_GEMM_NONE ? MVLT_OK : launch_tn(p, *a, (hipStream_t)stream);
 }
 
+extern "C" int mvlt_nn_version(void) { return MVLT_NN_VERSION; }
+extern "C" int mvlt_gemm_nn_sizeof(void) { return (int)sizeof(mvlt_gemm_nn_args); }
+extern "C" int mvlt_gemm_nn_plan(const mvlt_gemm_nn_args* q, mvlt_gemm_plan* plan) {
+  MVLT_REQUIRE(q && plan, "mvlt_gemm_nn_plan: null argument");
+  return plan_gemm_nn(*q, *plan);
+}
+extern "C" int mvlt_gemm_nn(const mvlt_gemm_nn_args* q, void* stream) {
+  mvlt_gemm_plan p;
+  MVLT_REQUIRE(q, "mvlt_gemm_nn: null operand");
+  if (int e = plan_gemm_nn(*q, p)) return e;
+  return p.family == MVLT_GEMM_NONE ? MVLT_OK : mvlt_launch_nn_dma(p, q->nt, q->b_rows, (hipStream_t)stream);
+}
+
 extern "C" int mvlt_plan_version(void) { return MVLT_PLAN_VERSION; }
 extern "C" int mvlt_gemm_plan_sizeof(void) { return (int)sizeof(mvlt_gemm_plan); }
 extern "C" int mvlt_gemm_nt_plan(const mvlt_gemm_nt_args* a, mvlt_gemm_plan* plan) {
diff --git a/mvlt_amd/csrc/gemm_common.h b/mvlt_amd/csrc/gemm_common.h
--- a/mvlt_amd/csrc/gemm_common.h
+++ b/mvlt_amd/csrc/gemm_common.h
@@ -5,6 +5,7 @@
 #include "../../include/mvlt_hip.h"
 
 int mvlt_launch_nt_dma(const mvlt_gemm_plan& p, const mvlt_gemm_nt_args& a, hipStream_t s);
+int mvlt_launch_nn_dma(const mvlt_gemm_plan& p, const mvlt_gemm_nt_args& a, int b_rows, hipStream_t s);
 int mvlt_launch_nt_p8(const mvlt_gemm_plan& p, const mvlt_gemm_nt_args& a, hipStream_t s);
 int mvlt_launch_nt_conv3(const mvlt_gemm_plan& p, const mvlt_gemm_nt_args& a, hipStream_t s);
 int mvlt_launch_tn_dma(const mvlt_gemm_plan& p, const mvlt_gemm_tn_args& k, bf16* part, hipStream_t s);
diff --git a/mvlt_amd/csrc/gemm_nt_dma.hip b/mvlt_amd/csrc/gemm_nt_dma.hip
--- a/mvlt_amd/csrc/gemm_nt_dma.hip
+++ b/mvlt_amd/csrc/gemm_nt_dma.hip
@@ -144,8 +144,8 @@
   nt_epilogue<T, BN>(p, acc, smem, m0, n0, wave, lane);
 }
 
-template <int BN, int AMODE, int EPI, int BK, int BMT = BM>
-__global__ __launch_bounds__(NTHREADS, BMT == 256 ? 2 : 1) void gemm_nt_dma_kernel(mvlt_gemm_nt_args p, int ns_flags) {
+template <int BN, int AMODE, int EPI, int BK, int BMT, bool BNN>
+__device__ __forceinline__ void gemm_nt_dma_body(const mvlt_gemm_nt_args& p, int ns_flags, int b_rows) {
   const int ns = ns_flags & 0xff;
   const bool early = (ns_flags & 0x100) != 0;
   constexpr int ROWB = BK * 2;
@@ -191,19 +191,30 @@
     a_y[i] = it.y; a_x[i] = it.x;
     a_ptr[i] = (const char*)p.A + (unsigned long long)(unsigned)phys * (2u * (unsigned)p.lda);
   }
+  using TB = DmaTile<BN>;
+  static_assert(!BNN || (BK == TBK && AMODE == 0 && BMT == BM && TB::IT == B_ITERS && TB::BYTES == BN * ROWB), "the NN form: 64-deep k-stages, plain rows, 128-row tiles");
   const char* b_ptr[B_ITERS];
   bool b_ok[B_ITERS];
+  const int b_row0 = tid / TB::CH;
+  const int b_k = b_rows > 0 ? b_rows : p.K;
 #pragma unroll
   for (int i = 0; i < B_ITERS; ++i) {
-    int n = n0 + row_in + RPL * i;
-    b_ok[i] = n < p.N;
-    b_ptr[i] = (const char*)p.B + (unsigned long long)(unsigned)(b_ok[i] ? n : 0) * (2u * (unsigned)p.ldb);
+    if constexpr (BNN) {
+      const int n = n0 + (((tid % TB::CH) ^ (TB::h(b_row0) << 1)) << 3);
+      b_ok[i] = n < p.N;
+      b_ptr[i] = (const char*)p.B + (unsigned long long)(unsigned)(b_row0 + TB::RPP * i) * (2u * (unsigned)p.ldb) + 2u * (unsigned)(b_ok[i] ? n : 0);
+    } else {
+      int n = n0 + row_in + RPL * i;
+      b_ok[i] = n < p.N;
+      b_ptr[i] = (const char*)p.B + (unsigned long long)(unsigned)(b_ok[i] ? n : 0) * (2u * (unsigned)p.ldb);
+    }
   }
 
   const int nk_all = (p.K + BK - 1) / BK;
   const int nsplit = p.split_k > 1 ? p.split_k : 1;
   const int kt_per = (nk_all + nsplit - 1) / nsplit;
   const int kt0 = blockIdx.y * kt_per;
+  int kbase = kt0 * BK;
   int kpos = kt0 * BK + chunk * 8, seg = 0, kk = kpos;
   if constexpr (AMODE != 0) { seg = kk / amap.c_seg; kk -= seg * amap.c_seg; }
   auto issue = [&](int slot) {
@@ -222,10 +233,14 @@
       glds16(ok ? a_ptr[i] + off_bytes : zsrc, __builtin_amdgcn_readfirstlane(smem_lds + slot * STAGE + (i * NTHREADS + wave * 64) * 16));
     }
 #pragma unroll
-    for (int i = 0; i < B_ITERS; ++i)
-      glds16((b_ok[i] && k_ok) ? b_ptr[i] + kpos * 2 : zsrc,
-             __builtin_amdgcn_readfirstlane(smem_lds + slot * STAGE + BMT * ROWB + (i * NTHREADS + wave * 64) * 16));
+    for (int i = 0; i < B_ITERS; ++i) {
+      const char* src;
+      if constexpr (BNN) src = (b_ok[i] && kbase + b_row0 + TB::RPP * i < b_k) ? b_ptr[i] + (unsigned long long)(unsigned)kbase * (2u * (unsigned)p.ldb) : zsrc;
+      else src = (b_ok[i] && k_ok) ? b_ptr[i] + kpos * 2 : zsrc;
+      glds16(src, __builtin_amdgcn_readfirstlane(smem_lds + slot * STAGE + BMT * ROWB + (i * NTHREADS + wave * 64) * 16));
+    }
     kpos += BK;
+    kbase += BK;
     if constexpr (AMODE != 0) {
       kk += BK;
       while (kk >= amap.c_seg) { kk -= amap.c_seg; ++seg; }
@@ -241,6 +256,9 @@
   const int nk = min(kt_per, nk_all - kt0);
   if (nk <= 0) return;
   const int fr = lane & 15, fg = lane >> 4;
+  int boff[TN_];
+#pragma unroll
+  for (int j = 0; j < TN_; ++j) boff[j] = BNN ? TB::frag_off(8 * fg + (fr >> 2), wn * TN_ + j, fr) : 0;
   for (int st = 0; st < (early ? ns : ns - 1) && st < nk; ++st) issue(st);
   if (ns == 1 && !early) issue(0);
   int slot = 0, islot = early ? 0 : ns - 1;
@@ -258,7 +276,7 @@
       islot = islot + 1 >= ns ? 0 : islot + 1;
     }
     const char* a_s = smem + slot * STAGE + (wm * WM) * ROWB;
-    const char* b_s = smem + slot * STAGE + BMT * ROWB + (wn * WN) * ROWB;
+    const char* b_s = smem + slot * STAGE + BMT * ROWB + (BNN ? 0 : (wn * WN) * ROWB);
     slot = slot + 1 >= ns ? 0 : slot + 1;
     constexpr int KS = BK / 32;
     u32x4 fa[KS][TM_], fb[KS][TN_];
@@ -272,7 +290,8 @@
 #pragma unroll
       for (int j = 0; j < TN_; ++j) {
         int r = j * 16 + fr;
-        fb[ks][j] = *(const u32x4*)(b_s + r * ROWB + swzk(wn * WN + r, ks * 4 + fg) * 16);
+        if constexpr (BNN) fb[ks][j] = tr_frag(b_s + boff[j] + ks * 32 * TB::ROWB, TB::ROWB);
+        else fb[ks][j] = *(const u32x4*)(b_s + r * ROWB + swzk(wn * WN + r, ks * 4 + fg) * 16);
       }
     }
     if (early) {
@@ -296,6 +315,15 @@
   if constexpr (BN == 192) nt_epilogue_192<EPI>(p, acc, smem, m0, n0, wave, lane);
   else if constexpr (EPI == 0) nt_epilogue<bf16, BN>(p, acc, smem, m0, n0, wave, lane);
   else nt_epilogue_lean<BN, EPI, TM_>(p, acc, smem, m0, n0, wave, lane);
+}
+
+template <int BN, int AMODE, int EPI, int BK, int BMT = BM>
+__global__ __launch_bounds__(NTHREADS, BMT == 256 ? 2 : 1) void gemm_nt_dma_kernel(mvlt_gemm_nt_args p, int ns_flags) {
+  gemm_nt_dma_body<BN, AMODE, EPI, BK, BMT, false>(p, ns_flags, 0);
+}
+template <int BN, int EPI>
+__global__ __launch_bounds__(NTHREADS, 1) void gemm_nn_dma_kernel(mvlt_gemm_nt_args p, int ns_flags, int b_rows) {
+  gemm_nt_dma_body<BN, 0, EPI, TBK, BM, true>(p, ns_flags, b_rows);
 }
 
 }
@@ -317,3 +345,14 @@
   }
   return no_instantiation(who, p);
 }
+
+int mvlt_launch_nn_dma(const mvlt_gemm_plan& p, const mvlt_gemm_nt_args& a, int b_rows, hipStream_t s) {
+  const char* const who = "mvlt_gemm_nn";
+  MVLT_PLAN_LAUNCH_HEAD;
+#define NN_DMA(BN_, EPI_) MVLT_CASE(false, (gemm_nn_dma_kernel<BN_, EPI_>), (MVLT_GEMM_NT_DMA, BN_, 0, EPI_, 64, 1), a, p.ns_flags, b_rows)
+  switch (key) {
+    NN_DMA(64, 0) NN_DMA(64, 1) NN_DMA(64, 2) NN_DMA(64, 4)
+    NN_DMA(128, 0) NN_DMA(128, 1) NN_DMA(128, 2) NN_DMA(128, 4)
+  }
+  return no_instantiation(who, p);
+}
diff --git a/mvlt_amd/csrc/gemm_plan.h b/mvlt_amd/csrc/gemm_plan.h
--- a/mvlt_amd/csrc/gemm_plan.h
+++ b/mvlt_amd/csrc/gemm_plan.h
@@ -2,6 +2,7 @@
 #include <stdint.h>
 #include <stdio.h>
 #include "../../include/mvlt_hip_plan.h"
+#include "../../include/mvlt_hip_nn.h"
 #include "plan_common.h"
 #ifndef MVLT_NT_EARLY_DEFAULT
 #define MVLT_NT_EARLY_DEFAULT 0x100
@@ -69,6 +70,24 @@
   const int lds_loop = 2 * (2 * (2 * hm * 16) + 64 * (hn0 + hn1)) * 128, lds_epi = 8 * 32 * (16 * (hn0 + hn1) + 4) * 4;
   set_tp(p, MVLT_GEMM_NT_P8, epi, hm, hn0, hn1, rag);
   set_launch(p, 8 * cdiv(cdiv(a.M, bmt), 8) * cdiv(a.N, bnt), 1, 1, 512, lds_loop > lds_epi ? lds_loop : lds_epi);
+}
+
+inline int nt_lean_epi(const mvlt_gemm_nt_args& a) {
+  int epi = 0;
+  const bool plain_epi = a.act == 0 && !a.R && !a.row_scale && !a.col_sum && !a.H && a.c_map.mode == 0;
+  const bool lean_ok = (a.c_map.mode == 0 || (a.c_map.mode == 1 && a.c_map.c_seg % 8 == 0)) && a.split_k <= 1 && (a.N % 8 == 0 || plain_epi) && a.ldc % 8 == 0 && al16(a.C) &&
+                       (!a.R || al16(a.R)) && (!a.H || al16(a.H)) && a.M < (1 << 24);
+  if (lean_ok && a.c_map.mode == 1) {
+    if (a.act == 0 && !a.col_sum && !a.R && !a.row_scale) epi = 6;
+    else if (a.act == 0 && !a.col_sum && a.R) epi = 7;
+  } else if (lean_ok) {
+    if (a.act == 1 && !a.R && !a.row_scale && !a.col_sum && a.out_dtype == 0) epi = 3;
+    else if (a.act == 2 && !a.R && !a.row_scale && !a.col_sum && a.out_dtype == 0) epi = 4;
+    else if (a.act == 0 && a.R && !a.col_sum) epi = 2;
+    else if (a.act == 0 && !a.R && !a.row_scale && a.col_sum) epi = 5;
+    else if (a.act == 0 && !a.R && !a.row_scale && !a.col_sum) epi = 1;
+  }
+  return epi;
 }
 
 }
@@ -119,20 +138,7 @@
     set_launch(p, gx, ksplit, 1, NTHREADS, lds < stage ? stage : lds);
     return MVLT_OK;
   }
-  int epi = 0;
-  const bool plain_epi = a.act == 0 && !a.R && !a.row_scale && !a.col_sum && !a.H && a.c_map.mode == 0;
-  const bool lean_ok = (a.c_map.mode == 0 || (a.c_map.mode == 1 && a.c_map.c_seg % 8 == 0)) && a.split_k <= 1 && (a.N % 8 == 0 || plain_epi) && a.ldc % 8 == 0 && al16(a.C) &&
-                       (!a.R || al16(a.R)) && (!a.H || al16(a.H)) && a.M < (1 << 24);
-  if (lean_ok && a.c_map.mode == 1) {
-    if (a.act == 0 && !a.col_sum && !a.R && !a.row_scale) epi = 6;
-    else if (a.act == 0 && !a.col_sum && a.R) epi = 7;
-  } else if (lean_ok) {
-    if (a.act == 1 && !a.R && !a.row_scale && !a.col_sum && a.out_dtype == 0) epi = 3;
-    else if (a.act == 2 && !a.R && !a.row_scale && !a.col_sum && a.out_dtype == 0) epi = 4;
-    else if (a.act == 0 && a.R && !a.col_sum) epi = 2;
-    else if (a.act == 0 && !a.R && !a.row_scale && a.col_sum) epi = 5;
-    else if (a.act == 0 && !a.R && !a.row_scale && !a.col_sum) epi = 1;
-  }
+  const int epi = nt_lean_epi(a);
   const int bk = (!narrow && a.a_map.mode == 0 && (epi == 3 || epi == 4) && a.K <= 512) ? 32 : 64;
   const int nk = bk == 32 ? cdiv(a.K, 32) : cdiv(cdiv(a.K, 64), ksplit);
   const int ns = nk < 2 ? nk : 2;
@@ -188,6 +194,30 @@
   }
   set_tp(p, MVLT_GEMM_NT_DMA, bn, a.a_map.mode, epi, bk);
   set_launch(p, gx, ksplit, 1, NTHREADS, lds);
+  return MVLT_OK;
+}
+
+inline int plan_gemm_nn(const mvlt_gemm_nn_args& q, mvlt_gemm_plan& p) {
+  using namespace mvlt_plan;
+  const mvlt_gemm_nt_args& a = q.nt;
+  if (int e = plan_gemm_nt(a, p)) return e;
+  p = mvlt_gemm_plan{};
+  MVLT_REQUIRE(a.dtype == 0, "mvlt_gemm_nn: bf16 operands only (the fp32 path multiplies by its W^T copy: mvlt_gemm_nt)");
+  MVLT_REQUIRE(a.a_map.mode == 0 && a.c_map.mode == 0, "mvlt_gemm_nn: plain or batch-strided rows only (no gather on A, no scatter on C)");
+  MVLT_REQUIRE(a.N % 8 == 0 && a.ldb >= a.N, "mvlt_gemm_nn: N must be a multiple of 8 and ldb (the pitch of a row of B = one k) must cover it");
+  MVLT_REQUIRE(q.b_rows >= 0 && q.b_rows <= a.K, "mvlt_gemm_nn: b_rows must lie in [0, K]");
+  MVLT_REQUIRE(!a.post_y && !a.col_sum && a.act != 1, "mvlt_gemm_nn: input-gradient epilogues only (generic, plain, residual, GELU'): no post_y, no column statistics, no GELU");
+  if (a.M == 0) return MVLT_OK;
+  const int bn = a.N <= 64 ? 64 : 128;
+  const int ksplit = a.split_k > 1 ? a.split_k : 1;
+  const int epi = nt_lean_epi(a);
+  const long stage = (long)4 * 32 * (bn / 2 + 4) * sizeof(float);
+  const int nk = cdiv(cdiv(a.K, 64), ksplit);
+  const int ns = nk < 2 ? nk : 2;
+  p.ns_flags = nk >= 2 ? ns | MVLT_NT_EARLY_DEFAULT : ns;
+  const long lds = (long)ns * (BM + bn) * ROW_BYTES;
+  set_tp(p, MVLT_GEMM_NT_DMA, bn, 0, epi, 64, 1);
+  set_launch(p, 8 * cdiv(cdiv(a.M, BM), 8) * cdiv(a.N, bn), ksplit, 1, NTHREADS, lds < stage ? stage : lds);
   return MVLT_OK;
 }
 
@@ -307,7 +337,9 @@
   switch (p.family) {
     case MVLT_GEMM_NONE: w = snprintf(buf, n, "%s", ""); break;
     case MVLT_GEMM_NT_F32: w = snprintf(buf, n, "gemm_nt_kernel<float, %d>", t[0]); break;
-    case MVLT_GEMM_NT_DMA: w = snprintf(buf, n, "gemm_nt_dma_kernel<%d, %d, %d, %d, 128>", t[0], t[1], t[2], t[3]); break;
+    case MVLT_GEMM_NT_DMA:
+      w = t[4] ? snprintf(buf, n, "gemm_nn_dma_kernel<%d, %d>", t[0], t[2]) : snprintf(buf, n, "gemm_nt_dma_kernel<%d, %d, %d, %d, 128>", t[0], t[1], t[2], t[3]);
+      break;
     case MVLT_GEMM_NT_P8: w = snprintf(buf, n, "gemm_nt_p8_kernel<%d, %d, %d, %d, %s>", t[0], t[1], t[2], t[3], tf[t[4] != 0]); break;
     case MVLT_GEMM_NT_CONV3: w = snprintf(buf, n, "conv3_nt_kernel<%d, %d, %d>", t[0], t[1], t[2]); break;
     case MVLT_GEMM_TN_PLAIN:
diff --git a/mvlt_amd/heads.py b/mvlt_amd/heads.py
--- a/mvlt_amd/heads.py
+++ b/mvlt_amd/heads.py
@@ -2,7 +2,7 @@
 
 from . import ops
 from ._lib import rowmap
-from .layers import StoreAccess, _empty, linear, linear_bwd
+from .layers import StoreAccess, _empty, linear, linear_bwd, linear_nn
 from .params import pool_zeros
 from .plan import _EVERY, WORD_TABLE, plan_unit
 from .pvlt import EPS_DEFAULT, VOCAB, VOCAB_LD
@@ -156,14 +156,13 @@
         db = _empty((1, VOCAB_LD), torch.float32, dev)
         ops.batch_sum(dl, db, R, 1, VOCAB_LD, 1, VOCAB_LD)
         P.g("mlm_head.bias").add_(db[0, :VOCAB])
-    wT = P.wT(WORD_TABLE)
     if dt == torch.bfloat16:
         dtr32 = pool_zeros((R, Hd), torch.float32, dev)
-        linear(dl, wT, dtr32, split_k=4)
+        linear_nn(dl, P.w(WORD_TABLE), dtr32, split_k=4)
         dtr = dtr32.to(dt)
     else:
         dtr = _empty((R, Hd), dt, dev)
-        linear(dl, wT, dtr)
+        linear(dl, P.wT(WORD_TABLE), dtr)
     de = _mlm_transform_bwd(model, dtr, sv_t, e, R, unit)
     _embed_ln_bwd(model, "mlm_head_embed", de, sv_e, A, a_map, R, dA, c_map if c_map is not None else a_map, accumulate, unit)
     S.announce_prefix("mlm_head_embed.", "mlm_head.")
diff --git a/mvlt_amd/layers.py b/mvlt_amd/layers.py
--- a/mvlt_amd/layers.py
+++ b/mvlt_amd/layers.py
@@ -47,6 +47,11 @@
     return ops.gemm_nt(x, W, y, _rows(x) if M is None else M, N, K, x.stride(-2), K, y.stride(-2), **epi)
 
 
+def linear_nn(dy, W, dx, M=None, **epi):
+    out, N = W.shape[0], W.numel() // W.shape[0]
+    return ops.gemm_nn(dy, W, dx, _rows(dy) if M is None else M, N, dy.shape[-1], dy.stride(-2), N, dx.stride(-2), b_rows=out, **epi)
+
+
 def linear_bwd(on, dy, x, gW, gb, wT=None, dx=None, M=None, *, fuse=False, tn=None, dy_map=None, x_map=None, dx_map=None, overwrite=False, **epi):
     if on:
         rows, N1 = _rows(dy) if M is None else M, gW.shape[0]
diff --git a/mvlt_amd/ops.py b/mvlt_amd/ops.py
--- a/mvlt_amd/ops.py
+++ b/mvlt_amd/ops.py
@@ -39,6 +39,15 @@
     return C_out
 
 
+def _gemm_nn_args(A, W, C_out, M, N, K, lda, ldb, ldc, *, b_rows=0, **kw):
+    return L.GemmNNArgs(nt=_gemm_nt_args(A, W, C_out, M, N, K, lda, ldb, ldc, **kw), b_rows=b_rows)
+
+
+def gemm_nn(A, W, C_out, *dims, **kw):
+    check(L.lib.mvlt_gemm_nn(C.byref(_gemm_nn_args(A, W, C_out, *dims, **kw)), stream_ptr()), "mvlt_gemm_nn")
+    return C_out
+
+
 class Plan:
 
     def __init__(self, plan_fn, args, cls=None, name_fn=None):
@@ -54,6 +63,10 @@
 
 def gemm_nt_plan(*args, **kw):
     return Plan(L.lib.mvlt_gemm_nt_plan, _gemm_nt_args(*args, **kw))
+
+
+def gemm_nn_plan(*args, **kw):
+    return Plan(L.lib.mvlt_gemm_nn_plan, _gemm_nn_args(*args, **kw))
 
 
 def gemm_tn_plan(*args, **kw):
diff --git a/mvlt_amd/params.py b/mvlt_amd/params.py
--- a/mvlt_amd/params.py
+++ b/mvlt_amd/params.py
@@ -127,6 +127,8 @@
 
 
 class FlatStore:
+
+    NATURAL_DGRAD = ("text_embeddings.word_embeddings.weight",)
 
     def __init__(self, module, compute_dtype):
         self.module = module
@@ -297,6 +299,9 @@
             blocks.append((dims[0] * dims[1] * dims[2] + 255) // 256)
 
         for name in transposed:
+            if self.C is not None and name in self.NATURAL_DGRAD:
+                self.extra.pop(name + "::T", None)
+                continue
             transpose(name)
         for name in list(conv_perm) + list(conv3):
             out, cin, kh, kw = self.master(name).shape
```

After: 13120, median of 6. About the same (+0.1%).
